# xmed-lab/GL-Fusion

Hardware: AMD Instinct MI355X
Metric: clips/sec fwd+bwd (B=4, 3 views x16x112x112) per GPU, weak scaling (higher is better)
Workload: dtype f32 (amax-scaled split-fp16 x3 MFMA, fp32 accumulate: fp32-equivalent); 1 GPU; C2: (B,V,T,H,W)=(4,3,16,112,112) per GPU, views 1/3/4, fp32 train() fwd + sum-BCE + bwd; global_batch_clips=4, frames_per_view_per_gpu=64, precision=f16x3, parallelism=single GPU, ranks_in_collective=1

## Files before the change

### gl-fusion_amd/csrc/gemm_common.h

```cpp
#pragma once
#include "glf_common.h"

namespace glf {
struct Geo { int n_img, hs, ws, hd, wd, kh, kw, stride, pad, dil; };

struct GemmArgs {
    const float* A; const float* B; const float* bias; float* C;
    int M, N, K, lda, ldb, ldc, taps;
    unsigned tap_mask;
    long long tap_stride_b;
    int gather;
    Geo g;
    long long bsa, bsb, bsc;
    float alpha;
    int accumulate, split;
    int tiles_m, tiles_n;
    int vec_a, vec_b;
    int rect;
    const float* amax_a; const float* amax_b;
    const float* zeros;
    float* amax_c;
    double* colstats;
    float* colmax;
    float* partial;
    unsigned long long* stamps;
    int a_presplit, b_presplit;
    int flags;
    int epi;
    const float* res; long long ld_res;
    int relu;
    const int* seg_tab;
    int seg_kx;
};

constexpr int SEG_MAX = 28, SEG_MAX_BANDS = 7, SEG_MAX_REGIONS = SEG_MAX_BANDS * SEG_MAX_BANDS;
constexpr int SEG_REGION_INTS = 8;
constexpr int SEG_TAB_REGIONS = 64, SEG_TAB_OFFS = SEG_TAB_REGIONS + SEG_REGION_INTS * SEG_MAX_REGIONS;
constexpr int SEG_TAB_INTS = SEG_TAB_OFFS + 2 * SEG_MAX;
static_assert(SEG_TAB_OFFS % 2 == 0, "segment offsets are 8-byte aligned");
constexpr int ZERO_PAGE_FLOATS = 1 << 18;


int precision();
int init_gemm_bf16s_attrs();
bool bf16s_rows_ok(const GemmArgs& a);
bool bf16s_tn_ok(const GemmArgs& a);
int launch_rows_bf16s(const GemmArgs& a, dim3 grid, bool gather, hipStream_t s);
int launch_tn_bf16s(const GemmArgs& a, dim3 grid, bool gather, hipStream_t s);
int init_gemm_f16s_attrs();
int launch_rows_f16s(const GemmArgs& a, dim3 grid, bool gather, int nprod, hipStream_t s);
int launch_tn_f16s(const GemmArgs& a, dim3 grid, bool gather, int nprod, hipStream_t s);
int init_gemm_f16s4_attrs();
bool use_f16s4(const GemmArgs& a);
int launch_rows_f16s4(const GemmArgs& a, dim3 grid, bool gather, int nprod, hipStream_t s);
int launch_amax(const float* x, long long rows, int cols, long long ld, int vec, float* out, hipStream_t s);
int launch_split_packed(const float* x, long long rows, int cols, long long ld, const float* amax, float* out, long long ldo, hipStream_t s);
float* amax_scratch(int n, hipStream_t s);
const float* zero_page();
bool f16s_rows_ok(const GemmArgs& a);
bool f16s_tn_ok(const GemmArgs& a);
int launch_rows_f16s_seg(const GemmArgs& a, const glf_gemm_params* p, int nprod, hipStream_t s);
}

namespace {
using glf::Geo;
using glf::GemmArgs;

typedef float f32x16 __attribute__((ext_vector_type(16)));

constexpr int BM = 128, BN = 128, BK = 32;
constexpr int LD_T = 129;
constexpr int LD_V = 132;
constexpr int NTHREADS = 256;

struct GeoS { int hs, ws, hd, wd, kw, stride, pad, dil; };

__device__ __forceinline__ int map_src(const int hs, const int ws, const int kw, const int stride, const int pad,
                                       const int dil, const int gather, int n, int y, int x, int tap) {
    const int ky = tap / kw, kx = tap - ky * kw;
    int sy, sx;
    if (gather == 1) {
        sy = y * stride - pad + ky * dil;
        sx = x * stride - pad + kx * dil;
        if ((unsigned)sy >= (unsigned)hs || (unsigned)sx >= (unsigned)ws) return -1;
    } else {
        sy = y + pad - ky * dil;
        sx = x + pad - kx * dil;
        if (sy < 0 || sx < 0) return -1;
        if (stride > 1) {
            if ((sy % stride) != 0 || (sx % stride) != 0) return -1;
            sy /= stride; sx /= stride;
        }
        if (sy >= hs || sx >= ws) return -1;
    }
    return (n * hs + sy) * ws + sx;
}

__device__ __forceinline__ float4 ld4(const float* p, int nvalid, bool vec) {
    if (nvalid >= 4 && vec) return *reinterpret_cast<const float4*>(p);
    float4 v = make_float4(0.f, 0.f, 0.f, 0.f);
    if (nvalid > 0) v.x = p[0];
    if (nvalid > 1) v.y = p[1];
    if (nvalid > 2) v.z = p[2];
    if (nvalid > 3) v.w = p[3];
    return v;
}

__host__ __device__ inline void tap_rect(int gather, int tap, int kw, int pad, int dil, int hs, int ws, int hd, int wd,
                                         int& y0, int& y1, int& x0, int& x1) {
    const int ky = tap / kw, kx = tap - ky * kw;
    const int oy = (gather == 1) ? pad - ky * dil : ky * dil - pad;
    const int ox = (gather == 1) ? pad - kx * dil : kx * dil - pad;
    y0 = oy > 0 ? oy : 0;           y1 = hs + oy < hd ? hs + oy : hd;
    x0 = ox > 0 ? ox : 0;           x1 = ws + ox < wd ? ws + ox : wd;
    if (y1 < y0) y1 = y0;
    if (x1 < x0) x1 = x0;
}

__host__ __device__ inline void axis_band(int gather, int b, int d, int h, int& lo, int& hi, unsigned& taps) {
    int e1 = d < h - d ? d : h - d, e2 = d < h - d ? h - d : d;
    e1 = e1 < 0 ? 0 : (e1 > h ? h : e1);
    e2 = e2 < 0 ? 0 : (e2 > h ? h : e2);
    lo = b == 0 ? 0 : (b == 1 ? e1 : e2);
    hi = b == 0 ? e1 : (b == 1 ? e2 : h);
    const unsigned first = gather == 1 ? 0b110u : 0b011u, last = gather == 1 ? 0b011u : 0b110u;
    taps = b == 0 ? first : (b == 2 ? last : (d <= h - d ? 0b111u : 0b010u));
}
__host__ __device__ inline void region_of(int gather, int r, int d, int hd, int wd, int& y0, int& y1, int& x0, int& x1, unsigned& mask) {
    const int cell = (int)((0x8620'7531'4ull >> (4 * r)) & 0xf);
    unsigned ty, tx;
    axis_band(gather, cell / 3, d, hd, y0, y1, ty);
    axis_band(gather, cell % 3, d, wd, x0, x1, tx);
    mask = 0;
    for (int ky = 0; ky < 3; ++ky)
        for (int kx = 0; kx < 3; ++kx)
            if (((ty >> ky) & 1u) && ((tx >> kx) & 1u)) mask |= 1u << (ky * 3 + kx);
}

__device__ __forceinline__ float4 keep_if(bool c, const float4 v) {
// ... 71 lines not shown
```

### gl-fusion_amd/csrc/gemm_f16s.hip

```cpp
#include "gemm_common.h"
#include "split_f16.h"
#include <cstdlib>
#include <cstring>
#include <mutex>
#include <vector>

namespace {
using glf::SEG_TAB_REGIONS; using glf::SEG_REGION_INTS; using glf::SEG_TAB_OFFS;

#define GLF_MFMA_F16(a, b, c) __builtin_amdgcn_mfma_f32_32x32x16_f16(a, b, c, 0, 0, 0)
#define GLF_ROW3(c0, c1, m0, m1, ah, al, b0h, b0l, b1h, b1l)  \
    c0 = GLF_MFMA_F16(ah, b0h, c0);                         \
    c1 = GLF_MFMA_F16(ah, b1h, c1);                         \
    if (NP == 3) {                                          \
        m0 = GLF_MFMA_F16(al, b0h, m0);                     \
        m1 = GLF_MFMA_F16(al, b1h, m1);                     \
        m0 = GLF_MFMA_F16(ah, b0l, m0);                     \
        m1 = GLF_MFMA_F16(ah, b1l, m1);                     \
    }

constexpr int BM8 = 256;
constexpr int NT8 = 512;
constexpr int WAVE_ROWS = 4;
#ifndef GLF_IL_ALL
// ... 1179 lines not shown
#if defined(GLF_STAMPS) && GLF_STAMPS == 2
    wg_t2 = __builtin_amdgcn_s_memtime();
#endif

    const bool atomic = !args.partial && ((p_split > 1) || p_accumulate);
    const int col_l = lane & 31, row_l = 4 * (lane >> 5);
    float cmax = 0.f;
    auto emit = [&](const f32x16& acc, int ti, int tj) {
        const int col = tn * BN + wn + 32 * tj + col_l;
        if (col >= pN) return;
#pragma unroll
        for (int r = 0; r < 16; ++r) {
            const int row = tm * TM8 + wm + 32 * ti + (r & 3) + 8 * (r >> 2) + row_l;
            if (row < pM) {
                float* dst = C + (long long)row * ldc_e + col;
                const float v = p_alpha * acc[r];
                if (atomic) atomicAdd(dst, v); else { *dst = v; cmax = fmaxf(cmax, fabsf(v)); }
            }
        }
    };
    emit(c00 + m00 * 0x1p-11f, 0, 0); emit(c01 + m01 * 0x1p-11f, 0, 1);
    emit(c10 + m10 * 0x1p-11f, 1, 0); emit(c11 + m11 * 0x1p-11f, 1, 1);
    if (args.amax_c && !atomic && !args.partial) {
#pragma unroll
        for (int o = 32; o > 0; o >>= 1) cmax = fmaxf(cmax, __shfl_xor(cmax, o, 64));
        if (lane == 0 && cmax > *reinterpret_cast<volatile float*>(args.amax_c))
            atomicMax(reinterpret_cast<unsigned*>(args.amax_c), __float_as_uint(cmax));
    }
#if defined(GLF_STAMPS) && GLF_STAMPS == 2
    if (args.stamps != nullptr && blockIdx.x == gridDim.x / 2 && blockIdx.z == 0 && blockIdx.y == 0) {
        __builtin_amdgcn_s_waitcnt(0);
        const unsigned long long wg_t3 = __builtin_amdgcn_s_memtime();
        if (lane == 0) {
            unsigned long long* d_ = args.stamps + 64 + wave * 4;
            d_[0] = wg_t0; d_[1] = wg_t1; d_[2] = wg_t2; d_[3] = wg_t3; if (wave == 0) args.stamps[63] = (unsigned long long)ntiles;
        }
    }
#endif
}

__global__ __launch_bounds__(256) void amax_kernel(const float* __restrict__ x, long long rows, int cols, long long ld,
                                                   int vec, unsigned* __restrict__ out) {
    const int c4n = vec ? cols >> 2 : 0;
    const long long total4 = rows * c4n;
    float m = 0.f;
    for (long long i = (long long)blockIdx.x * blockDim.x + threadIdx.x; i < total4; i += (long long)gridDim.x * blockDim.x) {
        const long long r = i / c4n;
        const int c = (int)(i - r * c4n) * 4;
        const float4 v = *reinterpret_cast<const float4*>(x + r * ld + c);
        m = fmaxf(fmaxf(m, fmaxf(fabsf(v.x), fabsf(v.y))), fmaxf(fabsf(v.z), fabsf(v.w)));
    }
    const int tail = cols - 4 * c4n;
    if (tail) {
        for (long long i = (long long)blockIdx.x * blockDim.x + threadIdx.x; i < rows * tail; i += (long long)gridDim.x * blockDim.x) {
            const long long r = i / tail;
            m = fmaxf(m, fabsf(x[r * ld + (cols - tail) + (int)(i - r * tail)]));
        }
    }
#pragma unroll
    for (int o = 32; o > 0; o >>= 1) m = fmaxf(m, __shfl_xor(m, o));
    __shared__ float sm[4];
    if ((threadIdx.x & 63) == 0) sm[threadIdx.x >> 6] = m;
    __syncthreads();
    if (threadIdx.x == 0) {
        m = fmaxf(fmaxf(sm[0], sm[1]), fmaxf(sm[2], sm[3]));
        if (m > 0.f) atomicMax(out, __float_as_uint(m));
    }
}

__global__ __launch_bounds__(256) void split_packed_kernel(const float* __restrict__ x, long long rows, int cols4, long long ld,
                                                           const float* __restrict__ amax, float* __restrict__ out, long long ldo) {
    float sc, inv;
    pow2_scale(amax, sc, inv);
    const long long total = rows * cols4;
    for (long long i = (long long)blockIdx.x * blockDim.x + threadIdx.x; i < total; i += (long long)gridDim.x * blockDim.x) {
        const long long r = i / cols4;
        const int c = (int)(i - r * cols4) * 4;
        const SplitH s = split4h(*reinterpret_cast<const float4*>(x + r * ld + c), sc);
        const float2 h = __builtin_bit_cast(float2, s.h), l = __builtin_bit_cast(float2, s.l);
        *reinterpret_cast<float4*>(out + r * ldo + c) = make_float4(h.x, h.y, l.x, l.y);
    }
}

}

namespace glf {

int launch_split_packed(const float* x, long long rows, int cols, long long ld, const float* amax, float* out, long long ldo, hipStream_t s) {
    const long long total = rows * (cols / 4);
    long long blocks = (total + 255) / 256;
    if (blocks > 8192) blocks = 8192;
    hipLaunchKernelGGL(split_packed_kernel, dim3((unsigned)blocks), dim3(256), 0, s, x, rows, cols / 4, ld, amax, out, ldo);
    return check_launch("split_f16_packed");
}

int init_gemm_f16s_attrs() {
    hipError_t e;
#define SET_ATTR(fn, bytes)                                                                              \
    e = hipFuncSetAttribute(reinterpret_cast<const void*>(fn), hipFuncAttributeMaxDynamicSharedMemorySize, (int)(bytes)); \
    if (e != hipSuccess) return fail(GLF_ERR_LAUNCH, "hipFuncSetAttribute(" #fn "): %s", hipGetErrorString(e));
#define SET_ROWS(G, NP_, PA_, PB_) SET_ATTR((gemm_rows_f16s8_kernel<G, NP_, PB_, PA_>), SMEM_ROWS_H8) SET_ATTR((gemm_rows_f16s8_kernel<G, NP_, PB_, PA_, true>), SMEM_ROWS_H8)
#define SET_TN(G, NP_, PA_, PB_) SET_ATTR((gemm_tn_f16s_kernel<G, NP_, PA_, PB_>), SMEM_TN_H) SET_ATTR((gemm_tn_f16s_kernel<G, NP_, PA_, PB_, true>), SMEM_TN_H) \
                                 SET_ATTR((gemm_tn_f16s8_kernel<G, NP_, PA_, PB_>), SMEM_TN_H8)
#define SET_ALL(G, NP_) SET_ROWS(G, NP_, false, false) SET_ROWS(G, NP_, true, false) SET_ROWS(G, NP_, false, true) SET_ROWS(G, NP_, true, true) \
                        SET_TN(G, NP_, false, false) SET_TN(G, NP_, true, false) SET_TN(G, NP_, false, true) SET_TN(G, NP_, true, true)
    SET_ALL(false, 3) SET_ALL(true, 3) SET_ALL(false, 1) SET_ALL(true, 1)
    SET_ATTR((gemm_rows_f16s8_kernel<false, 3, true, true, false, true>), SMEM_ROWS_H8)
    SET_ATTR((gemm_rows_f16s8_kernel<false, 1, true, true, false, true>), SMEM_ROWS_H8)
#undef SET_ALL
#undef SET_TN
#undef SET_ROWS
#undef SET_ATTR
    return init_gemm_f16s4_attrs();
}

bool f16s_rows_ok(const GemmArgs& a) {
    return a.vec_a && a.vec_b && (a.K % BK) == 0 && a.K >= BK && a.K <= ZERO_PAGE_FLOATS && zero_page() != nullptr;
}
bool f16s_tn_ok(const GemmArgs& a) {
    return a.vec_a && a.vec_b && (a.M % 4) == 0 && (a.N % 4) == 0 && a.M >= 4 && a.N >= 4 &&
           a.M <= ZERO_PAGE_FLOATS && a.N <= ZERO_PAGE_FLOATS && zero_page() != nullptr;
}

#ifdef GLF_STAMPS
static void* stamps_buffer() {
    static void* p = [] { void* q = nullptr; (void)hipMalloc(&q, 8192); (void)hipMemset(q, 0, 8192); return q; }();
    return p;
}
extern "C" int glf_debug_stamps(void* host_out) {
    (void)hipDeviceSynchronize();
    return (int)hipMemcpy(host_out, stamps_buffer(), 8192, hipMemcpyDeviceToHost);
}
#endif

int launch_rows_f16s(const GemmArgs& a0, dim3 grid, bool gather, int nprod, hipStream_t s) {
    if (use_f16s4(a0)) return launch_rows_f16s4(a0, grid, gather, nprod, s);
    GemmArgs a = a0;
    a.zeros = zero_page();
    long long tiles_m = (a.M + BM8 - 1) / BM8;
    if (a.rect == 2) {
        tiles_m = 0;
        for (int r = 0; r < 9; ++r) {
            int y0, y1, x0, x1;
            unsigned rm;
            region_of(a.gather, r, a.g.dil, a.g.hd, a.g.wd, y0, y1, x0, x1, rm);
            if (rm & a.tap_mask) tiles_m += ((long long)a.g.n_img * (y1 - y0) * (x1 - x0) + BM8 - 1) / BM8;
        }
        if (tiles_m == 0) return GLF_OK;
    } else if (a.rect) {
        tiles_m = 0;
        for (unsigned mm = a.tap_mask; mm; mm &= mm - 1) {
            const int t = __builtin_ctz(mm);
            int y0, y1, x0, x1;
            tap_rect(a.gather, t, a.g.kw, a.g.pad, a.g.dil, a.g.hs, a.g.ws, a.g.hd, a.g.wd, y0, y1, x0, x1);
            tiles_m += ((long long)a.g.n_img * (y1 - y0) * (x1 - x0) + BM8 - 1) / BM8;
        }
    }
    a.tiles_m = (int)tiles_m;
    dim3 g2((unsigned)(tiles_m * a.tiles_n), 1, grid.z);
    const int group_m = (a.rect == 0 && a.tiles_n >= 8) ? 4 : 0;
    a.flags = (group_m & 0xff) << 8;
    const bool pa = a.a_presplit != 0, pb = a.b_presplit != 0;
#ifdef GLF_STAMPS
    a.partial = reinterpret_cast<float*>(stamps_buffer());
#endif
#define GLF_LAUNCH_ROWS(G, NP_, PA_, PB_)                                                                                  \
    { if (a.epi) hipLaunchKernelGGL((gemm_rows_f16s8_kernel<G, NP_, PB_, PA_, true>), g2, dim3(NT8), SMEM_ROWS_H8, s, a); \
      else hipLaunchKernelGGL((gemm_rows_f16s8_kernel<G, NP_, PB_, PA_>), g2, dim3(NT8), SMEM_ROWS_H8, s, a); }
#define GLF_ROWS_P(G, NP_)                                                                     \
    { if (pa && pb) GLF_LAUNCH_ROWS(G, NP_, true, true) else if (pa) GLF_LAUNCH_ROWS(G, NP_, true, false) \
      else if (pb) GLF_LAUNCH_ROWS(G, NP_, false, true) else GLF_LAUNCH_ROWS(G, NP_, false, false) }
    if (nprod == 3) { if (gather) GLF_ROWS_P(true, 3) else GLF_ROWS_P(false, 3) }
    else { if (gather) GLF_ROWS_P(true, 1) else GLF_ROWS_P(false, 1) }
#undef GLF_ROWS_P
#undef GLF_LAUNCH_ROWS
    return check_launch("gemm_nt(f16x3, 256x128)");
// ... 182 lines not shown
```

### gl-fusion_amd/csrc/gemm_f32.hip

```cpp
#include "gemm_common.h"

namespace {

#define GLF_LD(x) (x)
#define GLF_MMA_KTILE(LDA_, LDB_, a_s, b_s, MID)                                                              \
    {                                                                                                         \
        constexpr int NS_ = BK / 2, HEAD_ = NS_ - 4;                                                          \
        f32x16 t00 = {0}, t01 = {0}, t10 = {0}, t11 = {0};                                                    \
        float a0_[2], a1_[2], b0_[2], b1_[2];                                                                 \
        float ta0_[4], ta1_[4], tb0_[4], tb1_[4];                                                             \
        a0_[0] = GLF_LD((a_s)[0]); a1_[0] = GLF_LD((a_s)[32]); b0_[0] = GLF_LD((b_s)[0]); b1_[0] = GLF_LD((b_s)[32]); \
        _Pragma("unroll") for (int st = 0; st < HEAD_; ++st) {                                                \
            const int cur = st & 1, nxt = cur ^ 1;                                                            \
            if (st + 1 < HEAD_) {                                                                             \
                a0_[nxt] = GLF_LD((a_s)[(2 * st + 2) * LDA_]); a1_[nxt] = GLF_LD((a_s)[(2 * st + 2) * LDA_ + 32]); \
                b0_[nxt] = GLF_LD((b_s)[(2 * st + 2) * LDB_]); b1_[nxt] = GLF_LD((b_s)[(2 * st + 2) * LDB_ + 32]); \
            } else {                                                                                          \
                _Pragma("unroll") for (int q = 0; q < 4; ++q) {                                               \
                    ta0_[q] = GLF_LD((a_s)[(2 * (HEAD_ + q)) * LDA_]); ta1_[q] = GLF_LD((a_s)[(2 * (HEAD_ + q)) * LDA_ + 32]); \
                    tb0_[q] = GLF_LD((b_s)[(2 * (HEAD_ + q)) * LDB_]); tb1_[q] = GLF_LD((b_s)[(2 * (HEAD_ + q)) * LDB_ + 32]); \
                }                                                                                             \
            }                                                                                                 \
            __builtin_amdgcn_sched_barrier(0);              \
            t00 = __builtin_amdgcn_mfma_f32_32x32x2f32(a0_[cur], b0_[cur], t00, 0, 0, 0);                     \
// ... 716 lines not shown
    }
    if (amax_c) {
#pragma unroll
        for (int o = 32; o > 0; o >>= 1) cmax = fmaxf(cmax, __shfl_xor(cmax, o, 64));
        if ((threadIdx.x & 63) == 0 && cmax > 0.f) atomicMax(reinterpret_cast<unsigned*>(amax_c), __float_as_uint(cmax));
    }
}

constexpr size_t SMEM_ROWS_NT = (2 * BK * LD_T + 2 * BK * LD_T) * sizeof(float) + 16;
constexpr size_t SMEM_ROWS_NN = (2 * BK * LD_T + 2 * BK * LD_V) * sizeof(float) + 16;
constexpr size_t SMEM_TN = (4 * BK * LD_V) * sizeof(float) + 2 * 32 * sizeof(int);

}

namespace glf {
int init_gemm_attrs() {
    hipError_t e;
#define SET_ATTR(fn, bytes)                                                                              \
    e = hipFuncSetAttribute(reinterpret_cast<const void*>(fn), hipFuncAttributeMaxDynamicSharedMemorySize, (int)(bytes)); \
    if (e != hipSuccess) return fail(GLF_ERR_LAUNCH, "hipFuncSetAttribute(" #fn "): %s", hipGetErrorString(e));
    SET_ATTR((gemm_rows_kernel<0, false>), SMEM_ROWS_NT)
    SET_ATTR((gemm_rows_kernel<0, true>), SMEM_ROWS_NT)
    SET_ATTR((gemm_rows_kernel<1, false>), SMEM_ROWS_NN)
    SET_ATTR((gemm_rows_kernel<1, true>), SMEM_ROWS_NN)
    SET_ATTR((gemm_tn_kernel<false>), SMEM_TN)
    SET_ATTR((gemm_tn_kernel<true>), SMEM_TN)
#undef SET_ATTR
    if (int rc = init_gemm_bf16s_attrs()) return rc;
    return init_gemm_f16s_attrs();
}
}

namespace {
int self_amax(GemmArgs& a, const glf_gemm_params* p, bool tn, hipStream_t s) {
    if (a.amax_a && a.amax_b) return GLF_OK;
    float* slots = glf::amax_scratch(2, s);
    GLF_REQUIRE(slots != nullptr, GLF_ERR_WORKSPACE, "gemm(f16x3): no amax scratch");
    hipError_t e = hipMemsetAsync(slots, 0, 2 * sizeof(float), s);
    if (e != hipSuccess) return glf::fail(GLF_ERR_LAUNCH, "hipMemsetAsync(amax): %s", hipGetErrorString(e));
    const long long src_rows = p->gather ? (long long)p->n_img * p->hs * p->ws : 0;
    for (int b = 0; b < p->batch; ++b) {
        if (!a.amax_a) {
            const long long rows = tn ? p->K : (p->gather ? src_rows : p->M);
            const int cols = tn ? p->M : p->K;
            if (int rc = glf::launch_amax(a.A + b * a.bsa, rows, cols, p->lda, a.vec_a, slots, s)) return rc;
        }
        if (!a.amax_b) {
            if (tn) {
                const long long rows = p->gather ? src_rows : p->K;
                if (int rc = glf::launch_amax(a.B + b * a.bsb, rows, p->N, p->ldb, a.vec_b, slots + 1, s)) return rc;
            } else {
                for (unsigned mm = p->tap_mask; mm; mm &= mm - 1) {
                    const int t = __builtin_ctz(mm);
                    if (int rc = glf::launch_amax(a.B + b * a.bsb + t * a.tap_stride_b, p->N, p->K, p->ldb, a.vec_b, slots + 1, s)) return rc;
                }
            }
        }
    }
    if (!a.amax_a) a.amax_a = slots;
    if (!a.amax_b) a.amax_b = slots + 1;
    return GLF_OK;
}
}

extern "C" int glf_amax(const float* x, int64_t rows, int cols, int64_t ld, float* out, glf_stream_t stream) {
    if (int rc = glf::ensure_init()) return rc;
    GLF_REQUIRE(x && out, GLF_ERR_NULL, "amax: null argument");
    GLF_REQUIRE(rows > 0 && cols > 0 && ld >= cols, GLF_ERR_BAD_SHAPE, "amax: bad extents");
    hipError_t e = hipMemsetAsync(out, 0, sizeof(float), glf::S(stream));
    if (e != hipSuccess) return glf::fail(GLF_ERR_LAUNCH, "hipMemsetAsync(amax): %s", hipGetErrorString(e));
    return glf::launch_amax(x, rows, cols, ld, aligned16(x) && (ld % 4 == 0), out, glf::S(stream));
}

extern "C" int glf_split_f16_packed(const float* x, int64_t rows, int cols, int64_t ld, const float* amax, float* out, int64_t ldo,
                                    glf_stream_t stream) {
    if (int rc = glf::ensure_init()) return rc;
    GLF_REQUIRE(x && amax && out, GLF_ERR_NULL, "split_f16_packed: null argument");
    GLF_REQUIRE(rows > 0 && cols > 0 && cols % 4 == 0 && ld % 4 == 0 && ldo % 4 == 0 && ld >= cols && ldo >= cols, GLF_ERR_BAD_SHAPE,
                "split_f16_packed: cols and the row strides must be multiples of 4");
    GLF_REQUIRE(aligned16(x) && aligned16(out), GLF_ERR_BAD_SHAPE, "split_f16_packed: x and out must be 16-byte aligned");
    return glf::launch_split_packed(x, rows, cols, ld, amax, out, ldo, glf::S(stream));
}

constexpr int SK_COLS = 2;
__global__ __launch_bounds__(256) void gemm_skinny_nt_kernel(const float* __restrict__ A, const float* __restrict__ B, const float* __restrict__ bias,
                                                            float* __restrict__ C, int M, int N, int K, int lda, int ldb, int ldc, float alpha,
                                                            int accumulate, float* __restrict__ amax_c) {
    const int tid = threadIdx.x, kl = tid & 3, m = tid >> 2;
    const int n0 = blockIdx.x * SK_COLS;
    const float* a = A + (long long)min(m, M - 1) * lda + 4 * kl;
    const float* b[SK_COLS];
#pragma unroll
    for (int j = 0; j < SK_COLS; ++j) b[j] = B + (long long)min(n0 + j, N - 1) * ldb + 4 * kl;
    float acc[SK_COLS] = {};
    int k = 0;
    for (; k + 64 <= K; k += 64) {
        float4 av[4], bv[SK_COLS][4];
#pragma unroll
        for (int u = 0; u < 4; ++u) av[u] = *reinterpret_cast<const float4*>(a + k + 16 * u);
#pragma unroll
        for (int j = 0; j < SK_COLS; ++j)
#pragma unroll
            for (int u = 0; u < 4; ++u) bv[j][u] = *reinterpret_cast<const float4*>(b[j] + k + 16 * u);
#pragma unroll
        for (int j = 0; j < SK_COLS; ++j)
#pragma unroll
            for (int u = 0; u < 4; ++u)
                acc[j] += av[u].x * bv[j][u].x + av[u].y * bv[j][u].y + av[u].z * bv[j][u].z + av[u].w * bv[j][u].w;
    }
    for (; k < K; k += 16) {
        const float4 av = *reinterpret_cast<const float4*>(a + k);
#pragma unroll
        for (int j = 0; j < SK_COLS; ++j) {
            const float4 bv = *reinterpret_cast<const float4*>(b[j] + k);
            acc[j] += av.x * bv.x + av.y * bv.y + av.z * bv.z + av.w * bv.w;
        }
    }
    float cmax = 0.f;
#pragma unroll
    for (int j = 0; j < SK_COLS; ++j) {
        float v = acc[j];
        v += __shfl_xor(v, 1);
        v += __shfl_xor(v, 2);
        if (kl == 0 && m < M && n0 + j < N) {
            v = v * alpha + (bias ? bias[n0 + j] : 0.f);
            float* c = C + (long long)m * ldc + n0 + j;
            if (accumulate) v += *c;
            *c = v;
            cmax = fmaxf(cmax, fabsf(v));
        }
    }
    if (amax_c) {
#pragma unroll
        for (int o = 32; o > 0; o >>= 1) cmax = fmaxf(cmax, __shfl_xor(cmax, o));
        if ((tid & 63) == 0 && cmax > 0.f) atomicMax(reinterpret_cast<unsigned*>(amax_c), __float_as_uint(cmax));
    }
}

extern "C" int glf_gemm_nt(const float* A, const float* B, const float* bias, float* C,
                           const glf_gemm_params* p, glf_stream_t stream) {
    if (int rc = glf::ensure_init()) return rc;
    if (int rc = validate(p, A, B, C)) return rc;
    if (p->gather) GLF_REQUIRE((long long)p->n_img * p->hd * p->wd == p->M, GLF_ERR_BAD_SHAPE,
                               "gemm_nt: M (%d) != n_img*hd*wd", p->M);
    if (p->tap_mask == 0) return glf::fail(GLF_ERR_BAD_SHAPE, "gemm_nt: empty tap_mask");
    GemmArgs a = make_args(A, B, bias, C, p);
    const int prec = call_precision(p);
    a.vec_a = aligned16(A) && (p->lda % 4 == 0) && (p->batch_stride_a % 4 == 0);
    a.vec_b = aligned16(B) && (p->ldb % 4 == 0) && (p->batch_stride_b % 4 == 0) && (p->tap_stride_b % 4 == 0);
    dim3 grid(a.tiles_m * a.tiles_n, 1, p->batch);
    if (p->nseg != 0) {
        GLF_REQUIRE(p->nseg >= 1 && p->nseg <= GLF_SEG_MAX && p->seg != nullptr, GLF_ERR_UNSUPPORTED, "glf_gemm_nt: nseg must be in [1, %d] with a segment list", GLF_SEG_MAX);
        GLF_REQUIRE(prec >= 2 && glf::f16s_rows_ok(a) && p->a_presplit && p->b_presplit && p->amax_a && p->amax_b, GLF_ERR_UNSUPPORTED,
                    "glf_gemm_nt: segments need precision 3 / 4, the aligned fast path and both operands pre-split with their amax");
        GLF_REQUIRE(!p->gather && p->taps == 1 && !p->rect && !p->accumulate && !p->colstats && !p->colmax && p->batch == 1, GLF_ERR_UNSUPPORTED,
                    "glf_gemm_nt: segments extend a plain NT launch (no gather, rect, accumulate, colstats or batch)");
        GLF_REQUIRE(p->n_img > 0 && p->hd > 0 && p->wd > 0 && (long long)p->n_img * p->hd * p->wd == p->M && p->K <= p->lda && p->N <= p->ldc,
                    GLF_ERR_BAD_SHAPE, "glf_gemm_nt: segments need M (%d) == n_img*hd*wd, K <= lda and N <= ldc", p->M);
        GLF_REQUIRE(p->seg_kx >= BK && p->seg_kx % BK == 0 && (long long)p->K + (long long)p->nseg * p->seg_kx <= p->ldb &&
                    (long long)p->K + (long long)p->nseg * p->seg_kx + BK <= glf::ZERO_PAGE_FLOATS, GLF_ERR_UNSUPPORTED,
                    "glf_gemm_nt: segments need seg_kx %% 32 == 0 and K + nseg * seg_kx <= ldb, < 2^18");
        for (int i = 0; i < p->nseg; ++i)
            GLF_REQUIRE(p->seg[3 * i + 2] >= 0 && p->seg[3 * i + 2] % 4 == 0 && p->seg[3 * i + 2] + p->seg_kx <= p->lda, GLF_ERR_UNSUPPORTED,
                        "glf_gemm_nt: segment %d: acol must be a multiple of 4 with acol + seg_kx <= lda", i);
        return glf::launch_rows_f16s_seg(a, p, prec == 2 ? 3 : 1, glf::S(stream));
    }
// ... 194 lines not shown
```

### gl-fusion_amd/csrc/norm.hip

```cpp
#include "stream_common.h"
#include "split_f16.h"

using namespace glf;

namespace {

constexpr int RT = 256;
constexpr int MAX_SLICES = 1024;

__host__ __device__ inline int n_slices_c(int rows, int c) {
    int s = (rows + 31) / 32;
    int cap = 524288 / (c > 0 ? c : 1);
    if (cap < 128) cap = 128;
    if (cap > MAX_SLICES) cap = MAX_SLICES;
    return s < 1 ? 1 : (s > cap ? cap : s);
}

struct Coef { const float* mean; const float* invstd; const float* gamma; const float* beta; };

struct OpStats {
    const float* x; int ldx;
    __device__ void operator()(int r, int c, float4& a, float4& b) const {
        a = *reinterpret_cast<const float4*>(x + (long long)r * ldx + c);
        b = make_float4(a.x * a.x, a.y * a.y, a.z * a.z, a.w * a.w);
// ... 234 lines not shown
                const unsigned m = RM == 1 ? op.mask[row * op.c4 + cc] : 15u;
                fold(row, qa, qa2, qx, qy, m);
            }
        }
        const int ncol = tpr * 4;
        for (int pass = 0; pass < (cmax ? 2 : 1); ++pass) {
            if (rl < rpp) {
                const float4 u = pass == 0 ? sa : mg, v = pass == 0 ? sb : mx;
                float* d0 = sh + (0 * rpp + rl) * ncol + ct * 4;
                float* d1 = sh + (1 * rpp + rl) * ncol + ct * 4;
                d0[0] = u.x; d0[1] = u.y; d0[2] = u.z; d0[3] = u.w;
                d1[0] = v.x; d1[1] = v.y; d1[2] = v.z; d1[3] = v.w;
            }
            __syncthreads();
            for (int idx = tid; idx < 2 * ncol; idx += RT) {
                const int st = idx / ncol, col = idx - st * ncol;
                const int gc = cb * 4 + col;
                if (gc < c) {
                    if (pass == 0) {
                        double d = 0;
                        for (int q = 0; q < rpp; ++q) d += sh[(st * rpp + q) * ncol + col];
                        atomicAdd(sums + st * c + gc, d);
                    } else {
                        float m = 0.f;
                        for (int q = 0; q < rpp; ++q) m = fmaxf(m, sh[(st * rpp + q) * ncol + col]);
                        if (m > 0.f) atomicMax(reinterpret_cast<unsigned*>(cmax + st * c + gc), __float_as_uint(m));
                    }
                }
            }
            __syncthreads();
        }
    }
}

constexpr int FIN_CH = 16, FIN_LANES = 16;

__device__ __forceinline__ void fold_partials(const double* __restrict__ partial, int slices, int c, int ch, int lane,
                                              double& s, double& q, double* sh) {
    s = 0; q = 0;
    if (ch < c) {
        double s1 = 0, q1 = 0, s2 = 0, q2 = 0, s3 = 0, q3 = 0;
        int i = lane;
        for (; i + 3 * FIN_LANES < slices; i += 4 * FIN_LANES) {
            s += partial[(long long)i * c + ch];                     q += partial[(long long)(slices + i) * c + ch];
            s1 += partial[(long long)(i + FIN_LANES) * c + ch];      q1 += partial[(long long)(slices + i + FIN_LANES) * c + ch];
            s2 += partial[(long long)(i + 2 * FIN_LANES) * c + ch];  q2 += partial[(long long)(slices + i + 2 * FIN_LANES) * c + ch];
            s3 += partial[(long long)(i + 3 * FIN_LANES) * c + ch];  q3 += partial[(long long)(slices + i + 3 * FIN_LANES) * c + ch];
        }
        for (; i < slices; i += FIN_LANES) {
            s += partial[(long long)i * c + ch];
            q += partial[(long long)(slices + i) * c + ch];
        }
        s += (s1 + s2) + s3; q += (q1 + q2) + q3;
    }
    const int t = threadIdx.x;
    sh[t] = s; sh[256 + t] = q;
    __syncthreads();
    if (lane == 0) {
        for (int l = 1; l < FIN_LANES; ++l) { s += sh[t + l * FIN_CH]; q += sh[256 + t + l * FIN_CH]; }
    }
}

__global__ __launch_bounds__(256) void bn_stats_finalize(const double* __restrict__ partial, int slices, int c, int rows, float eps,
                                                         float momentum, float* mean, float* invstd, float* rmean, float* rvar, long long* nbt) {
    __shared__ double sh[512];
    const int cx = threadIdx.x % FIN_CH, lane = threadIdx.x / FIN_CH;
    const int ch = blockIdx.x * FIN_CH + cx;
    double s, q;
    fold_partials(partial, slices, c, ch, lane, s, q, sh);
    if (lane != 0 || ch >= c) return;
    if (ch == 0 && nbt) *nbt += 1;
    const double m = s / rows;
    double var = q / rows - m * m;
    if (var < 0) var = 0;
    mean[ch] = (float)m;
    invstd[ch] = (float)(1.0 / sqrt(var + (double)eps));
    if (rmean) {
        const double unb = rows > 1 ? var * rows / (rows - 1) : var;
        rmean[ch] = (1.f - momentum) * rmean[ch] + momentum * (float)m;
        rvar[ch] = (1.f - momentum) * rvar[ch] + momentum * (float)unb;
    }
}

__global__ __launch_bounds__(256) void sum_finalize(const double* __restrict__ partial, int slices, int c, float* out_a, float* out_b) {
    __shared__ double sh[512];
    const int cx = threadIdx.x % FIN_CH, lane = threadIdx.x / FIN_CH;
    const int ch = blockIdx.x * FIN_CH + cx;
    double s, q;
    fold_partials(partial, slices, c, ch, lane, s, q, sh);
    if (lane != 0 || ch >= c) return;
    if (out_a) out_a[ch] = (float)s;
    if (out_b) out_b[ch] = (float)q;
}

__global__ __launch_bounds__(256) void bnbwd_finalize(const double* __restrict__ partial, const float* __restrict__ pmax, int slices, int c,
                                                      const float* __restrict__ gamma, const float* __restrict__ invstd, float inv_n,
                                                      int training, float* out_a, float* out_b, float* __restrict__ bound,
                                                      float* __restrict__ keep) {
    __shared__ double sh[512];
    __shared__ float shm[512];
    const int cx = threadIdx.x % FIN_CH, lane = threadIdx.x / FIN_CH;
    const int ch = blockIdx.x * FIN_CH + cx;
    double s, q;
    fold_partials(partial, slices, c, ch, lane, s, q, sh);
    float mg = 0.f, mx = 0.f;
    if (ch < c) {
        float g1 = 0.f, x1 = 0.f, g2 = 0.f, x2 = 0.f, g3 = 0.f, x3 = 0.f;
        int i = lane;
        for (; i + 3 * FIN_LANES < slices; i += 4 * FIN_LANES) {
            mg = fmaxf(mg, pmax[(long long)i * c + ch]);                      mx = fmaxf(mx, pmax[(long long)(slices + i) * c + ch]);
            g1 = fmaxf(g1, pmax[(long long)(i + FIN_LANES) * c + ch]);        x1 = fmaxf(x1, pmax[(long long)(slices + i + FIN_LANES) * c + ch]);
            g2 = fmaxf(g2, pmax[(long long)(i + 2 * FIN_LANES) * c + ch]);    x2 = fmaxf(x2, pmax[(long long)(slices + i + 2 * FIN_LANES) * c + ch]);
            g3 = fmaxf(g3, pmax[(long long)(i + 3 * FIN_LANES) * c + ch]);    x3 = fmaxf(x3, pmax[(long long)(slices + i + 3 * FIN_LANES) * c + ch]);
        }
        for (; i < slices; i += FIN_LANES) {
            mg = fmaxf(mg, pmax[(long long)i * c + ch]);
            mx = fmaxf(mx, pmax[(long long)(slices + i) * c + ch]);
        }
        mg = fmaxf(fmaxf(mg, g1), fmaxf(g2, g3)); mx = fmaxf(fmaxf(mx, x1), fmaxf(x2, x3));
    }
    shm[threadIdx.x] = mg; shm[256 + threadIdx.x] = mx;
    __syncthreads();
    if (lane != 0 || ch >= c) return;
    for (int l = 1; l < FIN_LANES; ++l) { mg = fmaxf(mg, shm[threadIdx.x + l * FIN_CH]); mx = fmaxf(mx, shm[256 + threadIdx.x + l * FIN_CH]); }
    if (out_a) out_a[ch] = (float)s;
    if (out_b) out_b[ch] = (float)q;
    if (keep) { keep[ch] = (float)s; keep[c + ch] = (float)q; }
    const float k = fabsf(gamma[ch] * invstd[ch]);
    const float b = 1.0001f * k * (training ? mg + inv_n * (fabsf((float)s) + mx * fabsf((float)q)) : mg);
    if (b > 0.f && b < 3.0e38f) atomicMax(reinterpret_cast<unsigned*>(bound), __float_as_uint(b));
}

__global__ void bn_replay_kernel(const float* __restrict__ mean, const float* __restrict__ invstd, int rows, float eps, float momentum,
                                 float* rmean, float* rvar, long long* nbt, int c) {
    const int ch = blockIdx.x * blockDim.x + threadIdx.x;
    if (ch == 0 && nbt) *nbt += 1;
    if (ch >= c) return;
    const double is = (double)invstd[ch];
    double var = 1.0 / (is * is) - (double)eps;
    if (var < 0) var = 0;
    const double unb = rows > 1 ? var * rows / (rows - 1) : var;
    rmean[ch] = (1.f - momentum) * rmean[ch] + momentum * mean[ch];
    rvar[ch] = (1.f - momentum) * rvar[ch] + momentum * (float)unb;
}

__global__ void bn_eval_coeffs_kernel(const float* rm, const float* rv, float eps, float* mean, float* invstd, int c) {
    const int ch = blockIdx.x * blockDim.x + threadIdx.x;
    if (ch >= c) return;
    mean[ch] = rm[ch];
    invstd[ch] = 1.0f / sqrtf(rv[ch] + eps);
}

constexpr int APPLY_TPR = 16, APPLY_TPR_WIDE = 64;
constexpr int APPLY_MAXCOL = APPLY_TPR_WIDE * 4;

struct ColGrid { int tpr, cblocks, slices; };
inline ColGrid col_grid(int rows, int c) {
    const int c4 = c / 4;
    const int tpr = c4 >= APPLY_TPR_WIDE ? APPLY_TPR_WIDE : (c4 < APPLY_TPR ? c4 : APPLY_TPR);
    const int rpp = 256 / tpr;
    const int cblocks = (c4 + tpr - 1) / tpr;
    long long s = stream_grid((long long)rows * c4, 256) / cblocks;
    const int smax = (rows + rpp - 1) / rpp;
    if (s > smax) s = smax;
    if (s < 1) s = 1;
    return {tpr, cblocks, (int)s};
}
inline dim3 col_dim(const ColGrid& g) { return dim3((unsigned)g.slices * (unsigned)g.cblocks); }

struct ColLane { int cb, slice, cc, c0, r, r1, rpp; bool live; };
__device__ __forceinline__ ColLane col_lane(int rows, int c4, int tpr, int cblocks, int slices) {
    ColLane L;
    L.rpp = 256 / tpr;
    const int ct = threadIdx.x % tpr, rl = threadIdx.x / tpr;
    L.cb = blockIdx.x % cblocks; L.slice = blockIdx.x / cblocks;
    const int per = (rows + slices - 1) / slices;
    const int r0 = L.slice * per;
    L.r1 = min(rows, r0 + per);
    L.r = r0 + rl;
    L.cc = L.cb * tpr + ct; L.c0 = L.cc * 4;
    L.live = L.cc < c4 && rl < L.rpp;
    return L;
}

template <bool RES>
__device__ __forceinline__ float bn_apply_rows(const ColLane& L, const float* __restrict__ x, int ldx, const float* __restrict__ res, int ldr,
                                               float* __restrict__ y, int ldy, const float4 mu, const float4 is, const float4 ga, const float4 be,
                                               int c4, int relu, unsigned char* __restrict__ mask, bool packed, float sc) {
    float am = 0.f;
    const int c0 = L.c0, cc = L.cc, rpp = L.rpp;
    auto emit = [&](long long row, const float4 xx, const float4 rr) __attribute__((always_inline)) {
        float4 o = make_float4(bn_val(xx.x, mu.x, is.x, ga.x, be.x), bn_val(xx.y, mu.y, is.y, ga.y, be.y),
                               bn_val(xx.z, mu.z, is.z, ga.z, be.z), bn_val(xx.w, mu.w, is.w, ga.w, be.w));
        if (RES) { o.x += rr.x; o.y += rr.y; o.z += rr.z; o.w += rr.w; }
        if (mask) mask[row * c4 + cc] = (unsigned char)((o.x > 0.f) | ((o.y > 0.f) << 1) | ((o.z > 0.f) << 2) | ((o.w > 0.f) << 3));
        if (relu) { o.x = fmaxf(o.x, 0.f); o.y = fmaxf(o.y, 0.f); o.z = fmaxf(o.z, 0.f); o.w = fmaxf(o.w, 0.f); }
        if (packed) {
            const SplitH sp = split4h(o, sc);
            const float2 h = __builtin_bit_cast(float2, sp.h), l = __builtin_bit_cast(float2, sp.l);
            o = make_float4(h.x, h.y, l.x, l.y);
        } else {
            am = fmaxf(fmaxf(am, fmaxf(fabsf(o.x), fabsf(o.y))), fmaxf(fabsf(o.z), fabsf(o.w)));
        }
        *reinterpret_cast<float4*>(y + row * ldy + c0) = o;
    };
    int r = L.r;
    for (; r + 3 * rpp < L.r1; r += 4 * rpp) {
        float4 qx[4], qr[4];
#pragma unroll
        for (int u = 0; u < 4; ++u) {
            const long long row = r + u * rpp;
            qx[u] = *reinterpret_cast<const float4*>(x + row * ldx + c0);
            if (RES) qr[u] = *reinterpret_cast<const float4*>(res + row * ldr + c0);
// ... 226 lines not shown
    const long long base = (long long)row * c;
    float4 u[LN_NV];
    float s = 0.f;
#pragma unroll
    for (int v = 0; v < LN_NV; ++v) {
        const int cc = lane + 64 * v;
        if (cc < c4) {
            const int ch = cc * 4;
            const float4 ww = *reinterpret_cast<const float4*>(w + base + ch);
            const float4 xx = *reinterpret_cast<const float4*>(x + base + ch);
            const float4 mu = *reinterpret_cast<const float4*>(bn.mean + ch);
            const float4 is = *reinterpret_cast<const float4*>(bn.invstd + ch);
            const float4 ga = *reinterpret_cast<const float4*>(bn.gamma + ch);
            const float4 be = *reinterpret_cast<const float4*>(bn.beta + ch);
            u[v] = make_float4((ww.x - mu.x) * is.x * ga.x + be.x + xx.x, (ww.y - mu.y) * is.y * ga.y + be.y + xx.y,
                               (ww.z - mu.z) * is.z * ga.z + be.z + xx.z, (ww.w - mu.w) * is.w * ga.w + be.w + xx.w);
            s += (u[v].x + u[v].y) + (u[v].z + u[v].w);
        } else {
            u[v] = make_float4(0.f, 0.f, 0.f, 0.f);
        }
    }
    float mean, rstd;
    if (!BWD) {
        mean = wave_sum(s) / c;
        float q = 0.f;
#pragma unroll
        for (int v = 0; v < LN_NV; ++v)
            if (lane + 64 * v < c4) {
                const float a = u[v].x - mean, b = u[v].y - mean, cc2 = u[v].z - mean, d = u[v].w - mean;
                q += (a * a + b * b) + (cc2 * cc2 + d * d);
            }
        rstd = 1.0f / sqrtf(wave_sum(q) / c + eps);
        if (lane == 0) { row_mean[row] = mean; row_rstd[row] = rstd; }
        float am = 0.f;
#pragma unroll
        for (int v = 0; v < LN_NV; ++v) {
            const int cc = lane + 64 * v;
            if (cc < c4) {
                const int ch = cc * 4;
                const float4 g = *reinterpret_cast<const float4*>(ln_g + ch);
                const float4 b = *reinterpret_cast<const float4*>(ln_b + ch);
                const float4 o = make_float4((u[v].x - mean) * rstd * g.x + b.x, (u[v].y - mean) * rstd * g.y + b.y,
                                             (u[v].z - mean) * rstd * g.z + b.z, (u[v].w - mean) * rstd * g.w + b.w);
                *reinterpret_cast<float4*>(z + base + ch) = o;
                am = fmaxf(fmaxf(am, fmaxf(fabsf(o.x), fabsf(o.y))), fmaxf(fabsf(o.z), fabsf(o.w)));
            }
        }
        if (amax_out) {
#pragma unroll
            for (int o = 32; o > 0; o >>= 1) am = fmaxf(am, __shfl_xor(am, o, 64));
            if (lane == 0 && am > *reinterpret_cast<volatile float*>(amax_out)) atomicMax(reinterpret_cast<unsigned*>(amax_out), __float_as_uint(am));
        }
    } else {
        mean = row_mean[row]; rstd = row_rstd[row];
        float4 gz[LN_NV];
        float s1 = 0.f, s2 = 0.f;
#pragma unroll
        for (int v = 0; v < LN_NV; ++v) {
            const int cc = lane + 64 * v;
            if (cc < c4) {
                const int ch = cc * 4;
                const float4 d = *reinterpret_cast<const float4*>(dz + base + ch);
                const float4 g = *reinterpret_cast<const float4*>(ln_g + ch);
                gz[v] = make_float4(d.x * g.x, d.y * g.y, d.z * g.z, d.w * g.w);
                u[v] = make_float4((u[v].x - mean) * rstd, (u[v].y - mean) * rstd, (u[v].z - mean) * rstd, (u[v].w - mean) * rstd);
                s1 += (gz[v].x + gz[v].y) + (gz[v].z + gz[v].w);
                s2 += (gz[v].x * u[v].x + gz[v].y * u[v].y) + (gz[v].z * u[v].z + gz[v].w * u[v].w);
            } else {
                gz[v] = make_float4(0.f, 0.f, 0.f, 0.f);
            }
        }
        const float m1 = wave_sum(s1) / c, m2 = wave_sum(s2) / c;
#pragma unroll
        for (int v = 0; v < LN_NV; ++v) {
            const int cc = lane + 64 * v;
            if (cc < c4)
                *reinterpret_cast<float4*>(du + base + cc * 4) =
                    make_float4(rstd * (gz[v].x - m1 - u[v].x * m2), rstd * (gz[v].y - m1 - u[v].y * m2),
                                rstd * (gz[v].z - m1 - u[v].z * m2), rstd * (gz[v].w - m1 - u[v].w * m2));
        }
    }
}

template <class Op>
int launch_colreduce(Op op, int rows, int c, double* ws, hipStream_t s) {
    const int slices = n_slices_c(rows, c);
    const int c4 = c / 4, tpr = c4 < RT ? c4 : RT;
    hipLaunchKernelGGL((colreduce_kernel<Op>), dim3(slices, (c4 + tpr - 1) / tpr), dim3(RT), 0, s, op, rows, c, slices, ws);
    return glf::check_launch("colreduce");
}

}

extern "C" size_t glf_bn_workspace(int rows, int c) {
    return (size_t)3 * MAX_SLICES * (size_t)(c > 0 ? c : 0) + (size_t)2 * (c > 0 ? c : 0);
}

#define REQ_C4(c) GLF_REQUIRE((c) > 0 && ((c) % 4) == 0, GLF_ERR_BAD_SHAPE, "channel count must be a positive multiple of 4 (got %d)", (c))
#define REQ_LD(ld, name) GLF_REQUIRE(((ld) % 4) == 0, GLF_ERR_BAD_SHAPE, name " must be a multiple of 4")

extern "C" int glf_bn_stats(const float* x, int ldx, int rows, int c, float eps, float momentum,
                            float* mean, float* invstd, float* running_mean, float* running_var,
                            int64_t* num_batches_tracked, double* workspace, glf_stream_t s) {
    if (int rc = glf::ensure_init()) return rc;
    GLF_REQUIRE(x && mean && invstd && workspace, GLF_ERR_NULL, "bn_stats: null argument");
    GLF_REQUIRE(rows > 0, GLF_ERR_BAD_SHAPE, "bn_stats: rows must be > 0");
    REQ_C4(c); REQ_AL(x, "x"); REQ_LD(ldx, "ldx");
    GLF_REQUIRE((running_mean == nullptr) == (running_var == nullptr), GLF_ERR_NULL, "bn_stats: running_mean/var must both be set or both NULL");
    if (int rc = launch_colreduce(OpStats{x, ldx}, rows, c, workspace, glf::S(s))) return rc;
    hipLaunchKernelGGL(bn_stats_finalize, dim3((c + FIN_CH - 1) / FIN_CH), dim3(256), 0, glf::S(s), workspace, n_slices_c(rows, c), c, rows,
                       eps, momentum, mean, invstd, running_mean, running_var, reinterpret_cast<long long*>(num_batches_tracked));
    return glf::check_launch("bn_stats_finalize");
}

extern "C" int glf_bn_stats_from_sums(const double* sums, int rows, int c, float eps, float momentum, float* mean, float* invstd,
                                      float* running_mean, float* running_var, int64_t* num_batches_tracked, glf_stream_t s) {
    if (int rc = glf::ensure_init()) return rc;
    GLF_REQUIRE(sums && mean && invstd, GLF_ERR_NULL, "bn_stats_from_sums: null argument");
    GLF_REQUIRE(rows > 0 && c > 0, GLF_ERR_BAD_SHAPE, "bn_stats_from_sums: rows and c must be > 0");
    GLF_REQUIRE((running_mean == nullptr) == (running_var == nullptr), GLF_ERR_NULL, "bn_stats_from_sums: running_mean/var must both be set or both NULL");
    hipLaunchKernelGGL(bn_stats_finalize, dim3((c + FIN_CH - 1) / FIN_CH), dim3(256), 0, glf::S(s), sums, 1, c, rows,
                       eps, momentum, mean, invstd, running_mean, running_var, reinterpret_cast<long long*>(num_batches_tracked));
    return glf::check_launch("bn_stats_from_sums");
}

extern "C" int glf_bn_replay_running(const float* mean, const float* invstd, int rows, int c, float eps, float momentum,
                                     float* running_mean, float* running_var, int64_t* num_batches_tracked, glf_stream_t s) {
    if (int rc = glf::ensure_init()) return rc;
    GLF_REQUIRE(mean && invstd && running_mean && running_var, GLF_ERR_NULL, "bn_replay_running: null argument");
    GLF_REQUIRE(rows > 0 && c > 0, GLF_ERR_BAD_SHAPE, "bn_replay_running: rows and c must be > 0");
    hipLaunchKernelGGL(bn_replay_kernel, dim3((c + 255) / 256), dim3(256), 0, glf::S(s), mean, invstd, rows, eps, momentum,
                       running_mean, running_var, reinterpret_cast<long long*>(num_batches_tracked), c);
    return glf::check_launch("bn_replay_running");
}

extern "C" int glf_bn_eval_coeffs(const float* rm, const float* rv, float eps, float* mean, float* invstd, int c, glf_stream_t s) {
    GLF_REQUIRE(rm && rv && mean && invstd, GLF_ERR_NULL, "bn_eval_coeffs: null argument");
    GLF_REQUIRE(c > 0, GLF_ERR_BAD_SHAPE, "bn_eval_coeffs: c must be > 0");
    hipLaunchKernelGGL(bn_eval_coeffs_kernel, dim3((c + 255) / 256), dim3(256), 0, glf::S(s), rm, rv, eps, mean, invstd, c);
    return glf::check_launch("bn_eval_coeffs");
}

extern "C" int glf_bn_apply(const float* x, int ldx, const float* residual, int ldr, float* y, int ldy,
                            const float* mean, const float* invstd, const float* gamma, const float* beta,
                            int rows, int c, int relu, float* amax_out, uint8_t* relu_mask, glf_stream_t s) {
    if (int rc = glf::ensure_init()) return rc;
    GLF_REQUIRE(x && y && mean && invstd && gamma && beta, GLF_ERR_NULL, "bn_apply: null argument");
    GLF_REQUIRE(rows > 0, GLF_ERR_BAD_SHAPE, "bn_apply: rows must be > 0");
    REQ_C4(c); REQ_AL(x, "x"); REQ_AL(y, "y"); REQ_LD(ldx, "ldx"); REQ_LD(ldy, "ldy");
    if (residual) { REQ_AL(residual, "residual"); REQ_LD(ldr, "ldr"); }
    const ColGrid g = col_grid(rows, c);
#define GLF_BNF(RES_) hipLaunchKernelGGL((bn_apply_kernel<RES_>), col_dim(g), dim3(256), 0, glf::S(s), x, ldx, residual, ldr, y, ldy, \
                                         Coef{mean, invstd, gamma, beta}, rows, c / 4, g.tpr, g.cblocks, g.slices, relu, amax_out, relu_mask)
    if (residual) GLF_BNF(true); else GLF_BNF(false);
#undef GLF_BNF
    return glf::check_launch("bn_apply");
}

extern "C" int glf_bn_apply_from_sums(const float* x, int ldx, const float* residual, int ldr, float* y, int ldy, const double* sums,
                                      int rows, int c, float eps, float momentum, const float* gamma, const float* beta,
                                      float* mean, float* invstd, float* running_mean, float* running_var, int64_t* num_batches_tracked,
                                      int relu, float* amax_out, uint8_t* relu_mask, const float* colmax, glf_stream_t s) {
    if (int rc = glf::ensure_init()) return rc;
    GLF_REQUIRE(x && y && sums && mean && invstd && gamma && beta, GLF_ERR_NULL, "bn_apply_from_sums: null argument");
    GLF_REQUIRE(!colmax || (amax_out && !residual && y != x), GLF_ERR_BAD_SHAPE, "bn_apply_from_sums: the packed output (colmax) needs amax_out, no residual and y != x");
    GLF_REQUIRE(rows > 0, GLF_ERR_BAD_SHAPE, "bn_apply_from_sums: rows must be > 0");
    REQ_C4(c); REQ_AL(x, "x"); REQ_AL(y, "y"); REQ_LD(ldx, "ldx"); REQ_LD(ldy, "ldy");
    GLF_REQUIRE(c <= APPLY_MAX_C, GLF_ERR_UNSUPPORTED, "bn_apply_from_sums: C must be <= %d (use glf_bn_stats_from_sums + glf_bn_apply)", APPLY_MAX_C);
    GLF_REQUIRE((running_mean == nullptr) == (running_var == nullptr), GLF_ERR_NULL, "bn_apply_from_sums: running_mean/var must both be set or both NULL");
    if (residual) { REQ_AL(residual, "residual"); REQ_LD(ldr, "ldr"); }
    const ColGrid g = col_grid(rows, c);
#define GLF_BNF(RES_) hipLaunchKernelGGL((bn_apply_sums_kernel<RES_>), col_dim(g), dim3(256), 0, glf::S(s), x, ldx, residual, ldr, y, ldy, sums, rows, c, \
                                         eps, momentum, gamma, beta, mean, invstd, running_mean, running_var,                                      \
                                         reinterpret_cast<long long*>(num_batches_tracked), g.tpr, g.cblocks, g.slices, relu, amax_out, relu_mask, colmax)
    if (residual) GLF_BNF(true); else GLF_BNF(false);
#undef GLF_BNF
    return glf::check_launch("bn_apply_from_sums");
}

extern "C" int glf_bn_bwd(const float* dy, int lddy, const float* x, int ldx, const float* y, int ldy,
                          const float* mean, const float* invstd, const float* gamma, const float* beta,
                          float* dx, int lddx, float* dres, int lddres, float* dgamma, float* dbeta,
                          int rows, int c, int relu, int training, double* workspace, float* amax_out, int packed_dx,
                          const uint8_t* relu_mask, const float* dy2, int lddy2, double* fused_sums, glf_stream_t s) {
    if (int rc = glf::ensure_init()) return rc;
    GLF_REQUIRE(dy && x && mean && invstd && gamma && dx && (workspace || fused_sums), GLF_ERR_NULL, "bn_bwd: null argument");
    if (relu_mask) y = nullptr;
    GLF_REQUIRE(!packed_dx || amax_out, GLF_ERR_NULL, "bn_bwd: packed_dx needs amax_out (a zeroed device float that receives the bound the image is scaled with)");
    GLF_REQUIRE(!relu || y || beta || relu_mask, GLF_ERR_NULL, "bn_bwd: relu != 0 needs relu_mask, y (the forward output) or beta (to recompute its sign from x)");
    GLF_REQUIRE(rows > 0, GLF_ERR_BAD_SHAPE, "bn_bwd: rows must be > 0");
    REQ_C4(c); REQ_AL(dy, "dy"); REQ_AL(x, "x"); REQ_AL(dx, "dx"); REQ_LD(lddy, "lddy"); REQ_LD(ldx, "ldx"); REQ_LD(lddx, "lddx");
    if (relu && y) { REQ_AL(y, "y"); REQ_LD(ldy, "ldy"); }
    if (dres) { REQ_AL(dres, "dres"); REQ_LD(lddres, "lddres"); }
    if (dy2) { REQ_AL(dy2, "dy2"); REQ_LD(lddy2, "lddy2"); }
    const OpBnBwd op{dy, lddy, x, ldx, y, ldy, mean, invstd, gamma, beta, relu, relu_mask, c / 4, dy2, lddy2};
    const ColGrid ag = col_grid(rows, c);
    BwdApply ap{dy, lddy, x, ldx, y, ldy, Coef{mean, invstd, gamma, beta}, nullptr, nullptr, dx, lddx, dres, lddres,
                rows, c, ag.tpr, ag.cblocks, ag.slices, training, 1.0f / (float)rows,
                amax_out, packed_dx, relu_mask, dy2, lddy2, nullptr, nullptr, nullptr, nullptr};
    const int phase = packed_dx >= 2 ? packed_dx : 0;
    GLF_REQUIRE(packed_dx >= 0 && packed_dx <= 3, GLF_ERR_BAD_SHAPE, "bn_bwd: packed_dx must be 0 .. 3");
    GLF_REQUIRE(!phase || (workspace && fused_sums), GLF_ERR_NULL, "bn_bwd: packed_dx = 2 / 3 needs the workspace and fused_sums (2 c floats kept from half 2 to half 3)");
    GLF_REQUIRE(phase != 2 || (dgamma && dbeta), GLF_ERR_NULL, "bn_bwd: packed_dx = 2 needs dgamma and dbeta");
    float* keep = phase ? reinterpret_cast<float*>(fused_sums) : (float*)nullptr;
    if (!phase && fused_sums && c <= APPLY_MAX_C) {
        float* fmax = reinterpret_cast<float*>(fused_sums + (size_t)2 * c);
        const int fs = fused_slices(rows, c);
        const int c4 = c / 4, tpr = c4 < FUSED_TPR ? c4 : FUSED_TPR;
        const dim3 rgrid(fs, (c4 + tpr - 1) / tpr);
        float* rmax = packed_dx ? fmax : (float*)nullptr;
        const int rm = !op.relu ? 0 : (op.mask ? 1 : (op.y ? 3 : 2));
        const bool wres = dy2 && dres;
        GLF_REQUIRE(!wres || (dres != dy && dres != dy2 && dres != x), GLF_ERR_BAD_SHAPE, "bn_bwd: dres must not alias dy, dy2 or x");
#define GLF_BNR(H2, RM_, WR) hipLaunchKernelGGL((bnbwd_reduce_atomic_kernel<H2, RM_, WR>), rgrid, dim3(RT), 0, glf::S(s), op, rows, c, fs, fused_sums, rmax, \
                                                (WR) ? dres : (float*)nullptr, lddres)
        if (wres) { if (rm == 0) GLF_BNR(true, 0, true); else if (rm == 1) GLF_BNR(true, 1, true); else if (rm == 2) GLF_BNR(true, 2, true); else GLF_BNR(true, 3, true); }
        else if (op.dy2) { if (rm == 0) GLF_BNR(true, 0, false); else if (rm == 1) GLF_BNR(true, 1, false); else if (rm == 2) GLF_BNR(true, 2, false); else GLF_BNR(true, 3, false); }
        else { if (rm == 0) GLF_BNR(false, 0, false); else if (rm == 1) GLF_BNR(false, 1, false); else if (rm == 2) GLF_BNR(false, 2, false); else GLF_BNR(false, 3, false); }
#undef GLF_BNR
        if (int rc = glf::check_launch("bn_bwd_reduce(fused)")) return rc;
        ap.fsums = fused_sums; ap.fmax = fmax; ap.out_dbeta = dbeta; ap.out_dgamma = dgamma;
        if (wres) {
            ap.dy = dres; ap.lddy = lddres; ap.dy2 = nullptr; ap.mask = nullptr; ap.y = nullptr; ap.dres = nullptr;
            return launch_bwd_apply(ap, 0, glf::S(s));
        }
        return launch_bwd_apply(ap, relu, glf::S(s));
    }
    GLF_REQUIRE(workspace, GLF_ERR_NULL, "bn_bwd: the three-launch form needs the workspace");
    const int slices = n_slices_c(rows, c);
    float* sums = reinterpret_cast<float*>(workspace + (size_t)2 * slices * c);
    float* s_dy = dbeta ? dbeta : sums;
    float* s_dyx = dgamma ? dgamma : sums + c;
    if (phase == 3) {
        s_dy = keep; s_dyx = keep + c;
    } else if (packed_dx) {
        float* pmax = reinterpret_cast<float*>(workspace + (size_t)2 * slices * c + (size_t)2 * c);
        const int c4 = c / 4, tpr = c4 < RT ? c4 : RT;
        hipLaunchKernelGGL(bnbwd_reduce_kernel, dim3(slices, (c4 + tpr - 1) / tpr), dim3(RT), 0, glf::S(s), op, rows, c, slices, workspace, pmax);
        if (int rc = glf::check_launch("bn_bwd_reduce")) return rc;
        hipLaunchKernelGGL(bnbwd_finalize, dim3((c + FIN_CH - 1) / FIN_CH), dim3(256), 0, glf::S(s), workspace, pmax, slices, c, gamma, invstd,
                           1.0f / (float)rows, training, s_dy, s_dyx, amax_out, keep);
    } else {
        if (int rc = launch_colreduce(op, rows, c, workspace, glf::S(s))) return rc;
        hipLaunchKernelGGL(sum_finalize, dim3((c + FIN_CH - 1) / FIN_CH), dim3(256), 0, glf::S(s), workspace, slices, c, s_dy, s_dyx);
    }
    if (int rc = glf::check_launch("bn_bwd_finalize")) return rc;
    if (phase == 2) return GLF_OK;
    ap.sum_dy = s_dy; ap.sum_dyx = s_dyx;
    return launch_bwd_apply(ap, relu, glf::S(s));
}

extern "C" int glf_colsum(const float* dy, int lddy, float* db, int rows, int c, double* workspace, glf_stream_t s) {
    if (int rc = glf::ensure_init()) return rc;
    GLF_REQUIRE(dy && db && workspace, GLF_ERR_NULL, "colsum: null argument");
    GLF_REQUIRE(rows > 0, GLF_ERR_BAD_SHAPE, "colsum: rows must be > 0");
    REQ_C4(c); REQ_AL(dy, "dy"); REQ_LD(lddy, "lddy");
    if (int rc = launch_colreduce(OpColsum{dy, lddy}, rows, c, workspace, glf::S(s))) return rc;
    hipLaunchKernelGGL(sum_finalize, dim3((c + FIN_CH - 1) / FIN_CH), dim3(256), 0, glf::S(s), workspace, n_slices_c(rows, c), c, db, (float*)nullptr);
    return glf::check_launch("colsum_finalize");
}

extern "C" int glf_bn_res_ln_fwd(const float* w, const float* x, const float* bn_mean, const float* bn_invstd,
                                 const float* bn_gamma, const float* bn_beta, const float* ln_gamma,
                                 const float* ln_beta, float ln_eps, float* z, float* row_mean, float* row_rstd,
                                 int rows, int c, float* amax_out, glf_stream_t s) {
    if (int rc = glf::ensure_init()) return rc;
    GLF_REQUIRE(w && x && bn_mean && bn_invstd && bn_gamma && bn_beta && ln_gamma && ln_beta && z && row_mean && row_rstd,
                GLF_ERR_NULL, "bn_res_ln_fwd: null argument");
    GLF_REQUIRE(rows > 0, GLF_ERR_BAD_SHAPE, "bn_res_ln_fwd: rows must be > 0");
    REQ_C4(c); GLF_REQUIRE(c <= 64 * 4 * LN_NV, GLF_ERR_UNSUPPORTED, "bn_res_ln: C must be <= %d", 64 * 4 * LN_NV);
    REQ_AL(w, "w"); REQ_AL(x, "x"); REQ_AL(z, "z");
    hipLaunchKernelGGL((bn_res_ln_kernel<false>), dim3((rows + 3) / 4), dim3(256), 0, glf::S(s), w, x,
                       Coef{bn_mean, bn_invstd, bn_gamma, bn_beta}, ln_gamma, ln_beta, ln_eps, z, row_mean, row_rstd,
                       (const float*)nullptr, (float*)nullptr, rows, c, amax_out);
    return glf::check_launch("bn_res_ln_fwd");
}

extern "C" int glf_bn_res_ln_bwd(const float* dz, const float* w, const float* x, const float* bn_mean,
                                 const float* bn_invstd, const float* bn_gamma, const float* bn_beta,
                                 const float* ln_gamma, const float* row_mean, const float* row_rstd,
                                 float* du, float* dln_gamma, float* dln_beta, int rows, int c,
                                 double* workspace, glf_stream_t s) {
    if (int rc = glf::ensure_init()) return rc;
    GLF_REQUIRE(dz && w && x && bn_mean && bn_invstd && bn_gamma && bn_beta && ln_gamma && row_mean && row_rstd && du &&
                dln_gamma && dln_beta && workspace, GLF_ERR_NULL, "bn_res_ln_bwd: null argument");
    GLF_REQUIRE(rows > 0, GLF_ERR_BAD_SHAPE, "bn_res_ln_bwd: rows must be > 0");
    REQ_C4(c); GLF_REQUIRE(c <= 64 * 4 * LN_NV, GLF_ERR_UNSUPPORTED, "bn_res_ln: C must be <= %d", 64 * 4 * LN_NV);
    REQ_AL(dz, "dz"); REQ_AL(w, "w"); REQ_AL(x, "x"); REQ_AL(du, "du");
    const Coef bn{bn_mean, bn_invstd, bn_gamma, bn_beta};
    hipLaunchKernelGGL((bn_res_ln_kernel<true>), dim3((rows + 3) / 4), dim3(256), 0, glf::S(s), w, x, bn, ln_gamma,
                       (const float*)nullptr, 0.f, (float*)nullptr, const_cast<float*>(row_mean), const_cast<float*>(row_rstd),
                       dz, du, rows, c, (float*)nullptr);
    if (int rc = glf::check_launch("bn_res_ln_bwd")) return rc;
    if (int rc = launch_colreduce(OpLnParam{dz, w, x, bn, row_mean, row_rstd, c}, rows, c, workspace, glf::S(s))) return rc;
    hipLaunchKernelGGL(sum_finalize, dim3((c + FIN_CH - 1) / FIN_CH), dim3(256), 0, glf::S(s), workspace, n_slices_c(rows, c), c, dln_gamma, dln_beta);
    return glf::check_launch("ln_param_finalize");
}
```

### gl-fusion_amd/fusion.py

```python
from __future__ import annotations

import ctypes as C
import os
import weakref
from types import SimpleNamespace

import torch
from torch.autograd import Function
from torch.autograd.function import once_differentiable

from ._lib import AttnPairParams, AttnParams, check, lib
from .ops import (_chk, _contig, _p, _stream, _tn_split, _ws, _wimage, _registry, WJ_COPY, stats_slot, bnbwd_slot, amax_of, amax_slot, colsum, gemm, set_amax, split_mode,
                  transpose2d, weight_T, weight_packed, nt_presplit_ok, tn_presplit_ok, act_packed, packed_hit, pick, zeros, _ones4)


FUSED_SOFTMAX = os.environ.get("GLF_FUSED_SOFTMAX", "1") != "0"
EXACT_KCHUNK = int(os.environ.get("GLF_EXACT_KCHUNK", "256"))
_gemm = gemm


def gemm(mode, A, B, Cm, **kw):
    K = kw["K"]
    if split_mode() or mode == "tn" or EXACT_KCHUNK <= 0 or K <= EXACT_KCHUNK or kw.get("taps", 1) != 1:
        return _gemm(mode, A, B, Cm, **kw)
    first = True
    for k0 in range(0, K, EXACT_KCHUNK):
        kk = dict(kw)
        kk["K"] = min(EXACT_KCHUNK, K - k0)
        if not first:
            kk["bias"] = None
            kk["accumulate"] = True
        _gemm(mode, A[..., k0:], B[..., k0:] if mode == "nt" else B[..., k0:, :], Cm, **kk)
        first = False
CHUNKED_SOFTMAX = os.environ.get("GLF_CHUNKED_SOFTMAX", "1") != "0"
CHUNK_BYTES = int(os.environ.get("GLF_SOFTMAX_CHUNK_BYTES", str(2 << 30)))


def chunked_softmax_ok(ci: int, L: int) -> bool:
    return CHUNKED_SOFTMAX and split_mode() and ci % 32 == 0 and L % 4 == 0


def gaussian_chunked_ok(ci: int) -> bool:
    return ci % 32 == 0


def pair_relu_ok(ci: int) -> bool:
    return ci % 32 == 0 and ci <= 1024


def _frames_per_chunk(n: int, L: int) -> int:
    lp = (L + 31) // 32 * 32
    return max(1, min(n, CHUNK_BYTES // (L * lp * 4)))


def _scores(th, ph, f0, g, L, lp, ci, c3, am_q, S):
    bq = L * c3
    gemm("nt", th[f0 * L:], ph[f0 * L:], S, M=L, N=L, K=ci, lda=c3, ldb=c3, ldc=lp, batch=g, bsa=bq, bsb=bq, bsc=L * lp,
         amax_a=am_q, amax_b=am_q)
    check(lib.glf_softmax_rows_ld(_p(S), g * L, L, lp, _stream()), "softmax_rows_ld")


def _transposed(src, f0, g, L, lp, ci, c3, out):
    check(lib.glf_transpose2d_strided(_p(src[f0 * L:]), c3, L * c3, _p(out), lp, ci * lp, L, ci, lp, g, _stream()), "transpose2d_strided")


def fused_softmax_ok(ci: int) -> bool:
    return FUSED_SOFTMAX and ci % 32 == 0 and ci <= 1024


def _pair_params(n: int, L: int, ci: int, ldg: int, ldy: int, lddy: int, lddg: int) -> AttnPairParams:
    pp = AttnPairParams()
    pp.frames, pp.L, pp.ci = n, L, ci
    pp.ldg, pp.ldy, pp.lddy, pp.lddg = ldg, ldy, lddy, lddg
    return pp


def _attn_params(n: int, L: int, ci: int, ldqkv: int, ldy: int) -> AttnParams:
    ap = AttnParams()
    ap.frames, ap.L, ap.ci = n, L, ci
    ap.ldq = ap.ldk = ap.ldv = ldqkv
    ap.ldy, ap.lddy, ap.ldd = ldy, ldy, ldqkv
    return ap


_qkv_cache = {}


def _qkv_weights(params):
    k = len(params) // 2
    ws_, bs_ = params[:k], params[k:]
    th_w = ws_[0]
    ci, c = th_w.shape[0], th_w.shape[1]
    if ci % 4 != 0:
        Wcat = torch.cat([_contig(t.detach()).view(ci, c) for t in ws_], dim=0)
        bcat = torch.cat([t.detach() for t in bs_], dim=0)
        return Wcat, bcat
    key = id(th_w)
    hit = _qkv_cache.get(key)
    if hit is None or hit[0]() is not th_w or hit[1].device != th_w.device or hit[1].shape != (k * ci, c):
        Wcat = torch.empty(k * ci, c, dtype=torch.float32, device=th_w.device)
# ... 205 lines not shown
        att = _full_softmax_fwd(G, (x2, x2, c, c, am_x), g, y)
    return y, att


def _gaussian_bwd(G, x, qkv, att, y, am_q, dy, am_dy, dqkv, am_dq_slot, du, wf):
    c, g = G.c, _slices(G, qkv)[2]
    x2 = x.view(G.rows, c)
    scores, sink = (x2, x2, c, c, amax_of(x)), (du, du, c, True, None)
    if gaussian_chunked_ok(G.ci):
        _group_softmax_bwd(G, scores, g, am_q, dy, am_dy, dqkv, am_dq_slot, sink)
    else:
        _full_softmax_bwd(G, scores, att, g, am_q, dy, am_dy, dqkv, sink)
    return None, None


def _concatenate_fwd(G, x, qkv, am_x, am_q, wf):
    n, L, ci, c3, rows = G.n, G.L, G.ci, G.c3, G.rows
    th, ph, g = _slices(G, qkv)
    wf_w, wf_b = wf
    if not pair_relu_ok(ci):
        raise RuntimeError(f"TPAVI mode 'concatenate' is built for Ci % 32 == 0, Ci <= 1024 (got {ci})")
    y = torch.empty(rows, ci, **G.f32)
    wrow = _contig(wf_w.detach()).view(2 * ci)
    att = torch.empty(2, rows, **G.f32)
    check(lib.glf_attn_pair_proj_fwd(_p(th), _p(ph), c3, _p(wrow), _p(att[0]), _p(att[1]), rows, ci, _stream()), "attn_pair_proj_fwd")
    pp = _pair_params(n, L, ci, c3, ci, ci, c3)
    check(lib.glf_attn_pair_relu_fwd(_p(att[0]), _p(att[1]), _p(wf_b), _p(g), _p(y), C.byref(pp), _stream()), "attn_pair_relu_fwd")
    return y, att


def _concatenate_bwd(G, x, qkv, att, y, am_q, dy, am_dy, dqkv, am_dq_slot, du, wf):
    n, L, ci, c3, rows = G.n, G.L, G.ci, G.c3, G.rows
    th, ph, g = _slices(G, qkv)
    dth, dph, dg = _slices(G, dqkv)
    wf_w, wf_b = wf
    wrow = _contig(wf_w.detach()).view(2 * ci)
    dab = torch.empty(2, rows, **G.f32)
    dwf_w = torch.empty(2 * ci, **G.f32)
    dwf_b = torch.empty(1, **G.f32)
    pp = _pair_params(n, L, ci, c3, ci, ci, c3)
    nb = int(lib.glf_attn_pair_relu_workspace_bytes(C.byref(pp)))
    ws = torch.empty(nb // 4, **G.f32)
    check(lib.glf_attn_pair_relu_bwd(_p(att[0]), _p(att[1]), _p(wf_b), _p(g), _p(dy), _p(dg), _p(dab[0]), _p(dab[1]), _p(dwf_b),
                                     _p(ws), nb, C.byref(pp), _stream()), "attn_pair_relu_bwd")
    nb = int(lib.glf_attn_pair_proj_workspace_bytes(rows, ci))
    ws = torch.empty(nb // 4, **G.f32)
    check(lib.glf_attn_pair_proj_bwd(_p(th), _p(ph), c3, _p(wrow), _p(dab[0]), _p(dab[1]), _p(dth), _p(dph), c3, _p(dwf_w), _p(ws), nb,
                                     rows, ci, _stream()), "attn_pair_proj_bwd")
    return dwf_w.view(wf_w.shape), dwf_b


_CORES = {"dot": (_dot_fwd, _dot_bwd), "embedded": (_embedded_fwd, _embedded_bwd), "gaussian": (_gaussian_fwd, _gaussian_bwd),
          "concatenate": (_concatenate_fwd, _concatenate_bwd)}


def _split_dgrad(G) -> bool:
    return split_mode() and G.ci % 32 == 0 and G.c % 32 == 0


def _project(G, x, Wcat, bcat):
    rows, c, c3 = G.rows, G.c, G.c3
    qkv = torch.empty(rows, c3, **G.f32)
    am_x = amax_of(x)
    am_q = amax_slot(G.dev)
    am_wc = amax_of(Wcat)
    ok = nt_presplit_ok(c, c, c)
    wb, pb = pick(Wcat, weight_packed(Wcat, Wcat, "w", am_wc) if ok else None, ok)
    xa, pa = pick(x, act_packed(x, am_x) if ok else None, ok)
    gemm("nt", xa, wb, qkv, M=rows, N=c3, K=c, lda=c, ldb=c, ldc=c3, bias=bcat, amax_a=am_x, amax_b=am_wc, amax_c=am_q,
         a_packed=pa, b_packed=pb)
    x_packed = (xa, am_x) if (pa and packed_hit(x, am_x) is not None) else None
    set_amax(qkv, am_q)
    return qkv, am_x, am_q, x_packed


def _project_bwd(G, x, dqkv, Wcat, du, x_packed):
    rows, c, c3 = G.rows, G.c, G.c3
    sp = _tn_split(rows, c3, c, 1)
    if not split_mode():
        sp = max(sp, min((rows + 511) // 512, 65535))
    dWcat = torch.empty(c3, c, **G.f32)
    am_dq = amax_of(dqkv)
    ok = tn_presplit_ok(c3, c, c3, c)
    dq_a, pa = pick(dqkv, act_packed(dqkv, am_dq, True) if ok else None, ok)
    am_x = x_packed[1] if x_packed is not None else amax_of(x)
    xb, pb = pick(x, x_packed[0] if x_packed is not None else None, ok)
    gemm("tn", dq_a, xb, dWcat, M=c3, N=c, K=rows, lda=c3, ldb=c, ldc=c, split=sp, amax_a=am_dq, amax_b=am_x, a_packed=pa, b_packed=pb)
    dbcat = colsum(dqkv, rows, c3)
    if _split_dgrad(G):
        WcatT = weight_T(Wcat, Wcat)
        am_wc = amax_of(Wcat)
        ok = nt_presplit_ok(c3, c3, c3)
        wb, pb = pick(WcatT, weight_packed(WcatT, Wcat, "T2", am_wc), ok)
        da, pa = pick(dqkv, act_packed(dqkv, am_dq, True) if ok else None, ok)
        gemm("nt", da, wb, du, M=rows, N=c, K=c3, lda=c3, ldb=c3, ldc=c, accumulate=True, amax_a=am_dq, amax_b=am_wc,
             a_packed=pa, b_packed=pb)
    else:
        gemm("nn", dqkv, Wcat, du, M=rows, N=c, K=c3, lda=c3, ldb=c, ldc=c, accumulate=True)
    return dWcat, dbcat


def _tail(G, x, y, zW, wz_w, wz_b, bn_g, bn_b, ln_g, ln_b, rmean, rvar, nbt, training, momentum, bn_eps, ln_eps):
    rows, c, ci, dev = G.rows, G.c, G.ci, G.dev
    wz = torch.empty(rows, c, **G.f32)
    am_zw = amax_of(wz_w)
    ok = nt_presplit_ok(ci, ci, ci)
    wb, pb = pick(zW, weight_packed(zW, wz_w, "w", am_zw) if ok else None, ok)
    am_y = amax_of(y)
    ya, pa = pick(y, act_packed(y, am_y) if ok else None, ok)
    fuse_stats = training and split_mode() and nt_presplit_ok(ci, ci, ci) and c % 4 == 0
    sums = stats_slot(c, dev) if fuse_stats else None
    gemm("nt", ya, wb, wz, M=rows, N=c, K=ci, lda=ci, ldb=ci, ldc=c, bias=wz_b, amax_a=am_y, amax_b=am_zw, a_packed=pa, b_packed=pb,
         colstats=sums)
    y_packed = (ya, am_y) if (pa and packed_hit(y, am_y) is not None) else None
    mean = torch.empty(c, **G.f32)
    invstd = torch.empty(c, **G.f32)
    if fuse_stats:
        check(lib.glf_bn_stats_from_sums(_p(sums), rows, c, bn_eps, momentum, _p(mean), _p(invstd), _p(rmean), _p(rvar), _p(nbt),
                                         _stream()), "bn_stats_from_sums")
    elif training:
        check(lib.glf_bn_stats(_p(wz), c, rows, c, bn_eps, momentum, _p(mean), _p(invstd), _p(rmean), _p(rvar), _p(nbt),
                               _p(_ws(rows, c, dev)), _stream()), "bn_stats")
    else:
        check(lib.glf_bn_eval_coeffs(_p(rmean), _p(rvar), bn_eps, _p(mean), _p(invstd), c, _stream()), "bn_eval_coeffs")
    z = torch.empty_like(x)
    rmu = torch.empty(rows, **G.f32)
    rrs = torch.empty(rows, **G.f32)
    am_z = amax_slot(dev)
    check(lib.glf_bn_res_ln_fwd(_p(wz), _p(x), _p(mean), _p(invstd), _p(bn_g), _p(bn_b), _p(ln_g), _p(ln_b), ln_eps,
                                _p(z), _p(rmu), _p(rrs), rows, c, _p(am_z), _stream()), "bn_res_ln_fwd")
    set_amax(z, am_z)
    return z, wz, mean, invstd, rmu, rrs, y_packed


def _tail_bwd(G, dz, x, y, wz, mean, invstd, rmu, rrs, zW, wz_o, bn_g, bn_b, ln_g, training, y_packed):
    rows, c, ci, dev = G.rows, G.c, G.ci, G.dev
    du = torch.empty(rows, c, **G.f32)
    dln_g = torch.empty(c, **G.f32)
    dln_b = torch.empty(c, **G.f32)
    check(lib.glf_bn_res_ln_bwd(_p(dz), _p(wz), _p(x), _p(mean), _p(invstd), _p(bn_g), _p(bn_b), _p(ln_g), _p(rmu), _p(rrs),
                                _p(du), _p(dln_g), _p(dln_b), rows, c, _p(_ws(rows, c, dev)), _stream()), "bn_res_ln_bwd")
    split = _split_dgrad(G)
    dwz = torch.empty(rows, c, **G.f32)
    am_dwz_slot = amax_slot(dev)
    dbn_g = torch.empty(c, **G.f32)
    dbn_b = torch.empty(c, **G.f32)
    dwz_pk = bool(training and split and am_dwz_slot is not None and nt_presplit_ok(c, c, c) and tn_presplit_ok(c, ci, c, ci))
    fused = bnbwd_slot(c, dev) if c <= 4096 else None
    check(lib.glf_bn_bwd(_p(du), c, _p(wz), c, None, c, _p(mean), _p(invstd), _p(bn_g), None, _p(dwz), c, None, c,
                         _p(dbn_g), _p(dbn_b), rows, c, 0, int(training), None if fused is not None else _p(_ws(rows, c, dev)), _p(am_dwz_slot),
                         int(dwz_pk), None, None, 0, _p(fused), _stream()), "bn_bwd")
    set_amax(dwz, am_dwz_slot)
    sp = _tn_split(rows, c, ci, 1)
    if not split_mode():
        sp = max(sp, min((rows + 511) // 512, 65535))
    dzW = torch.empty(c, ci, **G.f32)
    am_dwz = amax_of(dwz)
    ok = tn_presplit_ok(c, ci, c, ci)
    dwz_a, pa = (dwz, True) if dwz_pk else pick(dwz, act_packed(dwz, am_dwz, True) if ok else None, ok)
    am_y = y_packed[1] if y_packed is not None else amax_of(y)
    yb, pb = pick(y, y_packed[0] if y_packed is not None else None, ok)
    gemm("tn", dwz_a, yb, dzW, M=c, N=ci, K=rows, lda=c, ldb=ci, ldc=ci, split=sp, amax_a=am_dwz, amax_b=am_y, a_packed=pa, b_packed=pb)
    dzb = zeros(c, device=dev) if dwz_pk else colsum(dwz, rows, c)
    dy = torch.empty(rows, ci, **G.f32)
    if split:
        am_dy_slot = amax_slot(dev)
        zWT, am_zw = weight_T(zW, wz_o), amax_of(wz_o)
        ok = nt_presplit_ok(c, c, c)
        wb, pb = pick(zWT, weight_packed(zWT, wz_o, "T2", am_zw), ok)
        da, pa = (dwz, True) if dwz_pk else pick(dwz, act_packed(dwz, am_dwz, True) if ok else None, ok)
        gemm("nt", da, wb, dy, M=rows, N=ci, K=c, lda=c, ldb=c, ldc=ci, amax_a=am_dwz, amax_b=am_zw,
             amax_c=am_dy_slot, a_packed=pa, b_packed=pb)
        set_amax(dy, am_dy_slot)
    else:
        gemm("nn", dwz, zW, dy, M=rows, N=ci, K=c, lda=c, ldb=ci, ldc=ci)
    return du, dy, (dzW, dzb, dbn_g, dbn_b, dln_g, dln_b)


class TpaviFn(Function):
    @staticmethod
    def forward(ctx, x, th_w, th_b, ph_w, ph_b, g_w, g_b, wz_w, wz_b, bn_g, bn_b, ln_g, ln_b,
                rmean, rvar, nbt, training: bool, momentum: float, bn_eps: float, ln_eps: float, mode: str, wf_w=None, wf_b=None):
        x, G = _unpack(x, g_w, mode)
        zW = _contig(wz_w.detach()).view(wz_w.shape[0], wz_w.shape[1])
        Wcat, bcat = _qkv_weights((g_w, g_b) if G.npj == 1 else (th_w, ph_w, g_w, th_b, ph_b, g_b))
        qkv, am_x, am_q, ctx.x_packed = _project(G, x, Wcat, bcat)
        ctx.qkv_owner = g_w if G.npj == 1 else th_w
        ctx.wf = (wf_w, wf_b)
        y, att = _CORES[mode][0](G, x, qkv, am_x, am_q, ctx.wf)
        z, wz, mean, invstd, rmu, rrs, ctx.y_packed = _tail(G, x, y, zW, wz_w, wz_b, bn_g, bn_b, ln_g, ln_b, rmean, rvar, nbt,
                                                            training, momentum, bn_eps, ln_eps)
        ctx.save_for_backward(x, qkv, att, y, wz, mean, invstd, rmu, rrs, Wcat, zW, bn_g, bn_b, ln_g)
        ctx.cfg = (G.n, G.L, G.c, G.ci, training, mode, tuple(g_w.shape), tuple(wz_w.shape))
        ctx.owners = (wz_w,)
        return z

    @staticmethod
    @once_differentiable
    def backward(ctx, dz):
        (x, qkv, att, y, wz, mean, invstd, rmu, rrs, Wcat, zW, bn_g, bn_b, ln_g) = ctx.saved_tensors
        n, L, c, ci, training, mode, pshape, zshape = ctx.cfg
        G = _block(n, L, c, ci, mode, dz.device)
        du, dy, (dzW, dzb, dbn_g, dbn_b, dln_g, dln_b) = _tail_bwd(G, _contig(dz), x, y, wz, mean, invstd, rmu, rrs, zW, ctx.owners[0],
                                                                  bn_g, bn_b, ln_g, training, ctx.y_packed)
        dqkv = torch.empty(G.rows, G.c3, **G.f32)
        am_dq_slot = amax_slot(G.dev)
        dwf_w, dwf_b = _CORES[mode][1](G, x, qkv, att, y, amax_of(qkv), dy, amax_of(dy), dqkv, am_dq_slot, du, ctx.wf)
        del dy
        dWcat, dbcat = _project_bwd(G, x, dqkv, Wcat, du, ctx.x_packed)
        return _grads(G, x, du, dWcat, dbcat, pshape, dzW.view(zshape), dzb, dbn_g, dbn_b, dln_g, dln_b, dwf_w, dwf_b)


def tpavi_forward(x5: torch.Tensor, mod) -> torch.Tensor:
    bn = mod.W_z[1]
    training = bn.training
    if training and bn.momentum is None:
        raise RuntimeError("glfusion_amd: cumulative-average BatchNorm (momentum=None) is not built")
    fn = TpaviFn
    if x5.dtype == torch.bfloat16:
        from .fusion16 import Tpavi16Fn
        fn = Tpavi16Fn
    theta, phi = getattr(mod, "theta", None), getattr(mod, "phi", None)
    args = (x5, theta.weight if theta is not None else None, theta.bias if theta is not None else None,
            phi.weight if phi is not None else None, phi.bias if phi is not None else None, mod.g.weight, mod.g.bias,
            mod.W_z[0].weight, mod.W_z[0].bias, bn.weight, bn.bias, mod.norm_layer.weight, mod.norm_layer.bias,
            bn.running_mean, bn.running_var, bn.num_batches_tracked if training else None,
            training, float(bn.momentum or 0.0), float(bn.eps), float(mod.norm_layer.eps), mod.mode)
    wf = mod.W_f[0] if mod.mode == "concatenate" else None
    args += (wf.weight if wf is not None else None, wf.bias if wf is not None else None)
    return fn.apply(*args)
```

### gl-fusion_amd/ops.py

```python
from __future__ import annotations

import ctypes as C
import os
import weakref
from typing import List, Optional, Sequence, Tuple

import torch
from torch.autograd import Function
from torch.autograd.function import once_differentiable

from ._lib import GemmEpilogue, GemmParams, SEG_MAX, TN_OIHW_MAX_TAPS, WeightJob, WJ_AMAX, WJ_COPY, WJ_PACK, WJ_PASSES, WJ_PASS_OF, WJ_TAP_MAJOR, WJ_TAP_MAJOR_T, WJ_TRANSPOSE, WJ_ZERO, check, lib


BF = torch.bfloat16
DT_F32, DT_BF16 = 0, 1


def _is16(t) -> bool:
    return isinstance(t, torch.Tensor) and t.dtype == BF


def _p(t: Optional[torch.Tensor]):
    return None if t is None else C.c_void_p(t.data_ptr())

# ... 568 lines not shown
def weight_packed(layout: torch.Tensor, owner: torch.Tensor, tag: str, amax: Optional[torch.Tensor]) -> Optional[torch.Tensor]:
    if not presplit_ok(layout, amax):
        return None
    im, fresh = _wimage(owner, "pk:" + tag, WJ_PACK, layout, (layout.numel(), 0, 0), lambda: torch.empty_like(layout), amax)
    if fresh:
        cols = layout.shape[-1]
        check(lib.glf_split_f16_packed(_p(layout), layout.numel() // cols, cols, cols, _p(amax), _p(im.dst), cols, _stream()), "split_f16_packed")
    return im.dst


def packed_hit(t: torch.Tensor, amax: Optional[torch.Tensor]) -> Optional[torch.Tensor]:
    hit = getattr(t, "_glf_packed", None)
    if hit is not None and hit[0] == t._version and hit[1] == t.data_ptr() and hit[2] is amax:
        pk, made_on = hit[3], (hit[4] if len(hit) > 4 else None)
        if made_on is not None:
            cur = torch.cuda.current_stream()
            if made_on.cuda_stream != cur.cuda_stream:
                cur.wait_stream(made_on)
                pk.record_stream(cur)
        return pk
    share = getattr(t, "_glf_pack_share", None)
    if share is not None and share[0] is not None and share[0][0] == t.data_ptr() and share[0][1] is amax:
        pk, made_on = share[0][2], share[0][3]
        cur = torch.cuda.current_stream()
        if made_on.cuda_stream != cur.cuda_stream:
            cur.wait_stream(made_on)
            pk.record_stream(cur)
        return pk
    return None


PRESPLIT_KEEP_FRAC = float(os.environ.get("GLF_PRESPLIT_KEEP_FRAC", "0.5"))
PRESPLIT_OFF_FRAC = float(os.environ.get("GLF_PRESPLIT_OFF_FRAC", "0.6"))
_dev_total = {}
_retain_off = {}
_retain_step = {}


def retain_ok(dev) -> bool:
    hit = _retain_step.get(dev)
    if hit is not None:
        return hit
    tot = _dev_total.get(dev)
    if tot is None:
        tot = _dev_total[dev] = torch.cuda.get_device_properties(dev).total_memory
    off = _retain_off.get(dev, 0)
    if off:
        if off == 1 and torch.cuda.memory_allocated(dev) < 0.3 * tot and not torch.cuda.is_current_stream_capturing():
            torch.cuda.empty_cache()
            _retain_off[dev] = 2
        _retain_step[dev] = False
        return False
    r = torch.cuda.memory_reserved(dev)
    if r > PRESPLIT_OFF_FRAC * tot:
        _retain_off[dev] = 1
        _retain_step[dev] = False
        return False
    ok = r < PRESPLIT_KEEP_FRAC * tot
    if ok:
        _retain_step[dev] = True
    return ok


def act_packed(t: torch.Tensor, amax: Optional[torch.Tensor], retain: Optional[bool] = None) -> Optional[torch.Tensor]:
    if not presplit_ok(t, amax):
        return None
    pk = packed_hit(t, amax)
    if pk is not None:
        return pk
    pk = packed_of(t, amax)
    if retain is None:
        retain = retain_ok(t.device)
    if retain:
        try:
            t._glf_packed = (t._version, t.data_ptr(), amax, pk, torch.cuda.current_stream() if STREAMS else None)
        except AttributeError:
            pass
        share = getattr(t, "_glf_pack_share", None)
        if share is not None:
            share[0] = (t.data_ptr(), amax, pk, torch.cuda.current_stream())
    return pk


def nt_presplit_ok(K: int, lda: int, ldb: int) -> bool:
    return _PREC[0] >= 2 and K % 32 == 0 and 32 <= K <= (1 << 18) and lda % 4 == 0 and ldb % 4 == 0


def tn_presplit_ok(M: int, N: int, lda: int, ldb: int) -> bool:
    return _PREC[0] >= 2 and M % 4 == 0 and N % 4 == 0 and 4 <= M <= (1 << 18) and 4 <= N <= (1 << 18) and lda % 4 == 0 and ldb % 4 == 0


def pick(t: torch.Tensor, packed: Optional[torch.Tensor], ok: bool):
    return (packed, True) if (ok and packed is not None) else (t, False)


def weight_T(w2d: torch.Tensor, owner: torch.Tensor) -> torch.Tensor:
    rows, cols = w2d.shape
    src = _contig(w2d)
    im, fresh = _wimage(owner, "T2", WJ_TRANSPOSE, src, (rows, cols, 0),
                        lambda: torch.empty(cols, rows, dtype=torch.float32, device=owner.device))
    if fresh:
        check(lib.glf_transpose2d(_p(src), _p(im.dst), rows, cols, 1, _stream()), "transpose2d")
    return im.dst


def tap_major_T(weight: torch.Tensor) -> torch.Tensor:
    co, ci, kh, kw = weight.shape
    src = _contig(weight.detach())
    taps = kh * kw
    mk = lambda: torch.empty(taps, ci, co, dtype=torch.float32, device=weight.device)
    if taps == 1:
        im, fresh = _wimage(weight, "tapT", WJ_TRANSPOSE, src, (co, ci, 0), mk)
        if fresh:
            check(lib.glf_transpose2d(_p(src), _p(im.dst), co, ci, 1, _stream()), "transpose2d")
        return im.dst
    im, fresh = _wimage(weight, "tapT", WJ_TAP_MAJOR_T, src, (co, ci, taps), mk)
    if fresh:
        check(lib.glf_oihw_to_tap_major_t(_p(src), _p(im.dst), co, ci, taps, _stream()), "oihw_to_tap_major_t")
    return im.dst


def tap_major(weight: torch.Tensor) -> torch.Tensor:
    co, ci, kh, kw = weight.shape
    if kh * kw == 1:
        return _contig(weight.detach()).view(1, co, ci)
    src = _contig(weight.detach())
    im, fresh = _wimage(weight, "tap", WJ_TAP_MAJOR, src, (co, ci, kh * kw),
                        lambda: torch.empty(kh * kw, co, ci, dtype=torch.float32, device=weight.device))
    if fresh:
        check(lib.glf_oihw_to_tap_major(_p(src), _p(im.dst), co, ci, kh * kw, _stream()), "oihw_to_tap_major")
    return im.dst


_rect_cache = {}


def rect_fraction(gather: int, hd: int, wd: int, hs: int, ws: int, kh: int, kw: int, pad: int, dil: int, mask: int) -> float:
    key = (gather, hd, wd, hs, ws, kh, kw, pad, dil, mask)
    f = _rect_cache.get(key)
    if f is None:
        tot, n = 0, 0
        for t in range(kh * kw):
            if not (mask >> t) & 1:
                continue
            ky, kx = divmod(t, kw)
            oy = pad - ky * dil if gather == 1 else ky * dil - pad
            ox = pad - kx * dil if gather == 1 else kx * dil - pad
            rh = max(0, min(hs + oy, hd) - max(oy, 0))
            rw = max(0, min(ws + ox, wd) - max(ox, 0))
            tot += rh * rw
            n += 1
        f = tot / max(1, n * hd * wd)
        _rect_cache[key] = f
    return f


RECT_THRESHOLD = {"fwd": 0.8, "dgrad": 0.8, "wgrad": 0.8, "dgrad_f16x3": 0.35, "region": 0.8}


def region_mode(taps: int, kh: int, stride: int, pad: int, dil: int, h: int, w: int, ho: int, wo: int, k: int, frac: float) -> bool:
    return (_PREC[0] >= 2 and taps == 9 and kh == 3 and stride == 1 and pad == dil and h == ho and w == wo
            and k % 32 == 0 and frac < RECT_THRESHOLD["region"])


def _rect_thr(which: str) -> float:
    if which == "dgrad" and _PREC[0] >= 2:
# ... 1608 lines not shown
```

### include/glfusion.h

```cpp
#ifndef GLFUSION_H
#define GLFUSION_H

#include <stddef.h>
#include <stdint.h>

#ifdef __cplusplus
extern "C" {
#endif

typedef void* glf_stream_t;

typedef enum {
    GLF_OK = 0,
    GLF_ERR_BAD_SHAPE = -1,
    GLF_ERR_UNSUPPORTED = -2,
    GLF_ERR_WORKSPACE = -3,
    GLF_ERR_LAUNCH = -4,
    GLF_ERR_NULL = -5
} glf_status;

typedef enum { GLF_DT_F32 = 0, GLF_DT_BF16 = 1 } glf_dtype;

const char* glf_last_error(void);
int glf_abi_version(void);
int glf_init(void);
int glf_set_precision(int mode);
int glf_get_precision(void);
size_t glf_sizeof_gemm_params(void);

typedef struct {
    int32_t M, N, K;
    int32_t lda, ldb, ldc;
    int32_t taps;
    uint32_t tap_mask;
    int64_t tap_stride_b;
    int32_t gather;
    int32_t n_img, hs, ws, hd, wd, kh, kw, stride, pad, dil;
    int32_t batch;
    int64_t batch_stride_a, batch_stride_b, batch_stride_c;
    float alpha;
    int32_t accumulate;
    int32_t split;
    int32_t rect;
    const float* amax_a;
    const float* amax_b;
    float* amax_c;
    double* colstats;
    float* workspace;
    int64_t workspace_bytes;
    int32_t a_presplit;
    int32_t b_presplit;
    int32_t precision;
    float* colmax;
    int32_t c_dtype;
    int32_t reserved0;
    int32_t c_oihw;
    int32_t foreign_tap;
    const float* foreign_src;
    int64_t foreign_ld;
    int32_t nseg;
    int32_t seg_kx;
    int32_t* seg;
} glf_gemm_params;
#define GLF_TN_OIHW_MAX_TAPS 9
#define GLF_SEG_MAX 28
#define GLF_SEG_MAX_REGIONS 49
#define GLF_SEG_ROW_TILE 256

int glf_gemm_nt_seg_plan(int32_t n_img, int32_t h, int32_t w, int32_t nseg, const int32_t* seg, int32_t* regions,
                         int32_t* n_regions, int64_t* row_tiles);

int glf_amax(const float* x, int64_t rows, int cols, int64_t ld, float* out, glf_stream_t stream);
int glf_split_f16_packed(const float* x, int64_t rows, int cols, int64_t ld, const float* amax, float* out, int64_t ldo,
                         glf_stream_t stream);

int glf_gemm_nt(const float* A, const float* B, const float* bias, float* C,
                const glf_gemm_params* p, glf_stream_t stream);
int glf_gemm_nn(const float* A, const float* B, const float* bias, float* C,
                const glf_gemm_params* p, glf_stream_t stream);
int glf_gemm_tn(const float* A, const float* B, float* C,
                const glf_gemm_params* p, glf_stream_t stream);
size_t glf_gemm_tn_workspace_bytes(const glf_gemm_params* p);

typedef struct {
    const float* shift;
    const float* residual;
    int64_t ld_res;
    int32_t relu;
    int32_t reserved0;
} glf_gemm_epilogue;
int glf_gemm_nt_epilogue(const float* A, const float* B, float* C, const glf_gemm_params* p, const glf_gemm_epilogue* e,
                         glf_stream_t stream);

int glf_s16_gemm_nt(const void* A, const void* B, const float* bias, void* C, const glf_gemm_params* p, glf_stream_t stream);
int glf_s16_gemm_tn(const void* A, const void* B, void* C, const glf_gemm_params* p, glf_stream_t stream);
size_t glf_s16_gemm_tn_workspace_bytes(const glf_gemm_params* p);
typedef struct {
    const float* shift;
    const void* residual;
    int64_t ld_res;
    int32_t relu;
    int32_t reserved;
} glf_s16_gemm_epilogue;
int glf_s16_gemm_nt_epilogue(const void* A, const void* B, void* C, const glf_gemm_params* p, const glf_s16_gemm_epilogue* e,
                             glf_stream_t stream);

typedef struct {
    int32_t n, h, w, cin, cout, kh, kw, stride, pad, dil;
    int32_t precision;
    const float* amax_x;
    const float* amax_w;
    const float* amax_dy;
    float* amax_out;
    double* colstats;
} glf_conv_params;
typedef struct {
    int32_t ho, wo;
    int32_t M, N, K;
    int32_t taps, kept_taps;
    uint32_t tap_mask;
    int32_t plain;
    int32_t rect;
    int32_t split;
    int32_t zero_fill;
    int32_t colstats_ok;
    int64_t workspace_bytes;
} glf_conv_plan;
int glf_conv2d_plan(const glf_conv_params* p, int pass , glf_conv_plan* plan);
int glf_conv2d_fwd(const float* x, const float* w_tap, const float* bias, float* y, const glf_conv_params* p, glf_stream_t s);
int glf_conv2d_fwd_folded(const float* x, const float* w_tap_folded, const float* shift, const float* residual, int64_t ld_res,
                          int relu, float* y, const glf_conv_params* p, glf_stream_t s);
int glf_conv2d_dgrad(const float* dy, const float* w_tap, const float* w_tap_t, float* dx, const glf_conv_params* p, glf_stream_t s);
int glf_conv2d_wgrad(const float* dy, const float* x, float* dw_tap, float* workspace, int64_t workspace_bytes,
                     const glf_conv_params* p, glf_stream_t s);

typedef struct {
    int32_t frames, L, ci;
    int64_t ldq, ldk, ldv;
    int64_t ldy;
    int64_t lddy;
    int64_t ldd;
} glf_attn_params;
int glf_attn_softmax_fwd(const float* theta, const float* phi, const float* g, float* y, float* lse,
                         const glf_attn_params* p, glf_stream_t stream);
int glf_attn_softmax_bwd(const float* theta, const float* phi, const float* g, const float* y, const float* dy, const float* lse,
                         float* dtheta, float* dphi, float* dg, float* dsum_ws, const glf_attn_params* p, glf_stream_t stream);
int glf_s16_attn_softmax_fwd(const void* theta, const void* phi, const void* g, void* y, float* lse,
                             const glf_attn_params* p, glf_stream_t stream);
int glf_s16_attn_softmax_bwd(const void* theta, const void* phi, const void* g, const void* y, const void* dy,
                             const float* lse, void* dtheta, void* dphi, void* dg, float* dsum_ws,
                             const glf_attn_params* p, glf_stream_t stream);

typedef struct {
    int32_t frames, L, ci;
    int32_t reserved0;
    int64_t ldg;
    int64_t ldy;
// ... 115 lines not shown
} glf_tpavi_params;
size_t glf_sizeof_tpavi_params(void);
size_t glf_s16_tpavi_workspace_bytes(const glf_tpavi_params* p, int pass);
int glf_s16_tpavi_fwd(const void* x, const void* w_qkv, const float* b_qkv, const void* w_z, const float* b_z,
                      const float* bn_gamma, const float* bn_beta, float* bn_running_mean, float* bn_running_var,
                      int64_t* num_batches_tracked, const float* ln_gamma, const float* ln_beta, void* z,
                      void* qkv, void* att_t, void* y, void* wz, float* bn_mean, float* bn_invstd, float* row_mean, float* row_rstd,
                      const glf_tpavi_params* p, void* workspace, size_t workspace_bytes, glf_stream_t stream);
int glf_s16_tpavi_bwd(const void* dz, const void* x, const void* qkv, const void* att_t, const void* y, const void* wz,
                      const float* bn_mean, const float* bn_invstd, const float* row_mean, const float* row_rstd,
                      const void* w_qkv_t, const void* w_z_t, const float* bn_gamma, const float* bn_beta, const float* ln_gamma,
                      void* dx, float* dw_qkv, float* db_qkv, float* dw_z, float* db_z, float* dbn_gamma, float* dbn_beta,
                      float* dln_gamma, float* dln_beta, const glf_tpavi_params* p, void* workspace, size_t workspace_bytes,
                      glf_stream_t stream);

int glf_stem7x7_fwd(const float* x, const float* w, const float* bias, float* y,
                    int n, int h, int wdt, int cout, int pad, glf_stream_t s);
int glf_stem7x7_bn_relu_pool(const float* x, const float* w, const float* bias, const float* mean, const float* invstd,
                             const float* gamma, const float* beta, float* y, int n, int h, int wdt, int cout, int pad,
                             float* amax_out, glf_stream_t s);
size_t glf_stem7x7_wgrad_workspace(int n, int h, int wdt, int cout, int pad);
int glf_stem7x7_wgrad(const float* x, const float* dy, float* dw, float* db, float* partial,
                      int n, int h, int wdt, int cout, int pad, glf_stream_t s);

size_t glf_bn_workspace(int rows, int c);
int glf_bn_stats(const float* x, int ldx, int rows, int c, float eps, float momentum,
                 float* mean, float* invstd, float* running_mean, float* running_var,
                 int64_t* num_batches_tracked ,
                 double* workspace, glf_stream_t s);
int glf_bn_stats_from_sums(const double* sums, int rows, int c, float eps, float momentum, float* mean, float* invstd,
                           float* running_mean, float* running_var, int64_t* num_batches_tracked, glf_stream_t s);
int glf_bn_replay_running(const float* mean, const float* invstd, int rows, int c, float eps, float momentum,
                          float* running_mean, float* running_var, int64_t* num_batches_tracked, glf_stream_t s);
int glf_bn_eval_coeffs(const float* running_mean, const float* running_var, float eps,
                       float* mean, float* invstd, int c, glf_stream_t s);
int glf_bn_apply(const float* x, int ldx, const float* residual, int ldr, float* y, int ldy,
                 const float* mean, const float* invstd, const float* gamma, const float* beta,
                 int rows, int c, int relu, float* amax_out, uint8_t* relu_mask, glf_stream_t s);
int glf_bn_apply_from_sums(const float* x, int ldx, const float* residual, int ldr, float* y, int ldy, const double* sums,
                           int rows, int c, float eps, float momentum, const float* gamma, const float* beta,
                           float* mean, float* invstd, float* running_mean, float* running_var, int64_t* num_batches_tracked,
                           int relu, float* amax_out, uint8_t* relu_mask, const float* colmax, glf_stream_t s);
int glf_bn_bwd(const float* dy, int lddy, const float* x, int ldx, const float* y, int ldy,
               const float* mean, const float* invstd, const float* gamma, const float* beta ,
               float* dx, int lddx, float* dres, int lddres, float* dgamma, float* dbeta,
               int rows, int c, int relu, int training, double* workspace, float* amax_out, int packed_dx,
               const uint8_t* relu_mask , const float* dy2, int lddy2,
               double* fused_sums ,
               glf_stream_t s);

int glf_maxpool3x3s2_fwd(const float* x, float* y, uint8_t* idx, int n, int h, int w, int c, glf_stream_t s);
int glf_maxpool3x3s2_bwd(const float* dy, const uint8_t* idx, float* dx, int n, int h, int w, int c, glf_stream_t s);
int glf_avgpool_fwd(const float* x, float* y, int n, int p, int c, glf_stream_t s);
int glf_bcast_rows_fwd(const float* x, float* y, int ldy, int n, int p, int c, glf_stream_t s);
int glf_sum_rows_fwd(const float* dy, int lddy, float* dx, float scale, int n, int p, int c, glf_stream_t s);
int glf_bcast_rows_scaled(const float* x, float* y, int ldy, float scale, int n, int p, int c, glf_stream_t s);
int glf_bcast_rows_add(const float* x, float* y, int ldy, float scale, int n, int p, int c, glf_stream_t s);
int glf_relu_fwd(const float* x, float* y, int64_t numel, glf_stream_t s);
int glf_relu_bwd(const float* dy, const float* y, float* dx, int64_t numel, glf_stream_t s);
int glf_dropout(const float* x, float* y, int64_t numel, float p, uint64_t seed, const uint64_t* step_counter, glf_stream_t s);
int glf_amax_combine(const float* a, const float* b, float scale, int sum, float* out, glf_stream_t s);
int glf_counter_add(uint64_t* counter, uint64_t inc, glf_stream_t s);
int glf_gate_fwd(const float* cls, int ncls, const float* ctr, const float* f, float* y, float* a,
                 int32_t* argmax, float weight, int rows, int c, glf_stream_t s);
int glf_gate_bwd(const float* dy, const float* f, const float* cls, int ncls, const float* ctr,
                 const float* a, const int32_t* argmax, float weight,
                 float* df, float* dcls, float* dctr, int rows, int c, glf_stream_t s);
int glf_copy_frames(const float* src, int64_t src_fs, float* dst, int64_t dst_fs,
                    int n, int64_t inner, glf_stream_t s);
int glf_copy_frames_split(const float* src, int64_t src_fs, float* dst, float* dst_packed, int64_t dst_fs, int n, int64_t inner,
                          const float* amax, glf_stream_t s);
int glf_add_frames(const float* a, int64_t a_fs, const float* b, int64_t b_fs, float* dst, int64_t dst_fs,
                   int n, int64_t inner, glf_stream_t s);
int glf_add_n(const float* const* inputs, int k, float* out, int64_t numel, glf_stream_t s);
int glf_bn_res_ln_fwd(const float* w, const float* x, const float* bn_mean, const float* bn_invstd,
                      const float* bn_gamma, const float* bn_beta, const float* ln_gamma,
                      const float* ln_beta, float ln_eps, float* z, float* row_mean, float* row_rstd,
                      int rows, int c, float* amax_out, glf_stream_t s);
int glf_bn_res_ln_bwd(const float* dz, const float* w, const float* x, const float* bn_mean,
                      const float* bn_invstd, const float* bn_gamma, const float* bn_beta,
                      const float* ln_gamma, const float* row_mean, const float* row_rstd,
                      float* du, float* dln_gamma, float* dln_beta, int rows, int c,
                      double* workspace, glf_stream_t s);
int glf_softmax_rows(float* x, int64_t rows, int cols, glf_stream_t s);
int glf_softmax_rows_bwd(const float* p, float* dp_inout, int64_t rows, int cols, glf_stream_t s);
int glf_softmax_rows_ld(float* x, int64_t rows, int cols, int ld, glf_stream_t s);
int glf_softmax_rows_bwd_ld(const float* p, float* dp_inout, int64_t rows, int cols, int ld, glf_stream_t s);
int glf_bilinear_up_fwd(const float* x, float* y, int n, int h, int w, int c, int ho, int wo, glf_stream_t s);
int glf_bilinear_up_bwd(const float* dy, float* dx, int n, int h, int w, int c, int ho, int wo, glf_stream_t s);
int glf_bce_logits_sum(const float* x, const float* t, double* loss_out, float* dx, float grad_scale,
                       const float* grad_scale_dev, int64_t numel, glf_stream_t s);
int glf_overlap_counts(const float* logits, const float* target, int64_t* counts, int64_t numel, glf_stream_t s);
int glf_colsum(const float* dy, int lddy, float* db, int rows, int c, double* workspace, glf_stream_t s);

int glf_adam_step(const int64_t* table, int n_rows, double lr, double beta1, double beta2, double eps,
                  double weight_decay, int64_t step, glf_stream_t s);
int glf_sgd_step(const int64_t* table, int n_rows, double lr, double momentum, double dampening, double weight_decay,
                 int nesterov, int first, glf_stream_t s);
int glf_grad_sumsq(const int64_t* table, int n_rows, double* partials, glf_stream_t s);
int glf_grad_clip_coef(const double* partials, int n, double max_norm, float* record, int64_t* skipped, glf_stream_t s);
int glf_adam_step_clipped(const int64_t* table, int n_rows, double lr, double beta1, double beta2, double eps,
                          double weight_decay, int64_t step, const float* record, glf_stream_t s);
int glf_sgd_step_clipped(const int64_t* table, int n_rows, double lr, double momentum, double dampening, double weight_decay,
                         int nesterov, int first, const float* record, glf_stream_t s);
int glf_grad_scale(const int64_t* table, int n_rows, const float* record, glf_stream_t s);

int glf_seg_cycle(const float* feat, int T, int F, int target_region, int cyc_off, int chunk_size, float temperature,
                  int start0, int n_starts, int stride, float weight, int soft_label, float* loss_out, float* dfeat,
                  glf_stream_t s);
int glf_axpby(const float* x, const float* y, float* out, float a, float b, int64_t numel, glf_stream_t s);
int glf_scale(const float* x, float* y, int64_t numel, float scale, const float* scale_dev, glf_stream_t s);
int glf_prepare_frames(const float* img, const float* lab, float* out_img, float* out_mask, int H0, int W0, int T,
                       int resize, int out_h, int out_w, int off_y, int off_x, const int* class_to_channel, float img_div,
                       glf_stream_t s);
int glf_overlap_counts_nchw(const float* logits, const float* target, int64_t* counts, int n, int c, int64_t hw, glf_stream_t s);
int glf_zero(void* p, int64_t bytes, glf_stream_t s);

#ifdef __cplusplus
}
#endif
#endif
```

### profiles/ubench/kstats_groups.py

```python
#!/usr/bin/env python3
import csv
import re
import sys

rows = list(csv.DictReader(open(sys.argv[1])))
steps = float(sys.argv[2]) if len(sys.argv) > 2 else 1.0
groups = [("NT contractions", r"gemm_rows|s16_rows_kernel|gemm_skinny"), ("TN contractions (wgrad)", r"gemm_tn|s16_tn_kernel"), ("tn_reduce", r"tn_reduce"),
          ("BN bwd reduce", r"colreduce_kernel<.*OpBnBwd|bnbwd_reduce"), ("BN bwd apply", r"bn_bwd_apply|bnbwd_apply"), ("BN apply", r"bn_apply_kernel|bn_apply_sums"),
          ("BN stats / finalize", r"colreduce_kernel<.*OpStats|bn_stats_finalize|sum_finalize|bnbwd_finalize"),
          ("other column reduces", r"colreduce"), ("add_n (fan-in)", r"add_n"), ("split_packed", r"split_packed"),
          ("weights refresh", r"weights_refresh"), ("bn_res_ln", r"bn_res_ln"), ("stem", r"stem"), ("maxpool", r"maxpool"),
          ("at::native", r"at::native|elementwise_kernel|vectorized"), ("amax", r"amax_kernel")]
tot = {g: [0.0, 0] for g, _ in groups}
rest, rest_n, allt = {}, 0, 0.0
for r in rows:
    name, t, n = r["Name"], float(r["TotalDurationNs"]) / 1e6, int(r["Calls"])
    if re.search(r"spin_kernel|probe_mfma", name):
        aids = aids + t if "aids" in dir() else t
        continue
    allt += t
    for g, pat in groups:
        if re.search(pat, name):
            tot[g][0] += t; tot[g][1] += n
            break
    else:
        k = re.sub(r"\(anonymous namespace\)::|void ", "", name)[:50]
        rest[k] = rest.get(k, 0.0) + t
print(f"total kernel time {allt / steps:.1f} ms/step over {steps:g} steps (bench.py's spin / probe kernels left out: {(aids if 'aids' in dir() else 0.0) / steps:.1f} ms/step)")
for g, _ in groups:
    if tot[g][1]:
        print(f"  {g:28s} {tot[g][0] / steps:8.2f} ms/step  {tot[g][1] / steps:8.1f} launches/step")
for k, t in sorted(rest.items(), key=lambda kv: -kv[1])[:12]:
    print(f"  {k:50s} {t / steps:8.2f} ms/step")
```

Before: 17.51 clips/s.

## Fuse tail backward reductions and fold bias colsum into split-packed pass

Adds a fused bn_res_ln backward kernel that walks dz/w/x once. In that single pass it produces du plus the LN and BN column sums, and one merged finalize kernel reduces them. It also adds a split_packed_colsum kernel that computes the bias-gradient column sum while splitting the activation into fp16 hi/lo, so the separate colsum read of dqkv is gone. The intent is to cut memory passes and kernel launches in the transformer-tail backward. The cost is more complex kernels with higher register and shared-memory use, which may reduce occupancy, and a changed reduction order.

```diff
diff --git a/gl-fusion_amd/csrc/gemm_common.h b/gl-fusion_amd/csrc/gemm_common.h
--- a/gl-fusion_amd/csrc/gemm_common.h
+++ b/gl-fusion_amd/csrc/gemm_common.h
@@ -55,6 +55,8 @@
 int launch_rows_f16s4(const GemmArgs& a, dim3 grid, bool gather, int nprod, hipStream_t s);
 int launch_amax(const float* x, long long rows, int cols, long long ld, int vec, float* out, hipStream_t s);
 int launch_split_packed(const float* x, long long rows, int cols, long long ld, const float* amax, float* out, long long ldo, hipStream_t s);
+int launch_split_packed_colsum(const float* x, int rows, int cols, long long ld, const float* amax, float* out, long long ldo,
+                               float* colsum, double* workspace, hipStream_t s);
 float* amax_scratch(int n, hipStream_t s);
 const float* zero_page();
 bool f16s_rows_ok(const GemmArgs& a);
diff --git a/gl-fusion_amd/csrc/gemm_f16s.hip b/gl-fusion_amd/csrc/gemm_f16s.hip
--- a/gl-fusion_amd/csrc/gemm_f16s.hip
+++ b/gl-fusion_amd/csrc/gemm_f16s.hip
@@ -1285,6 +1285,79 @@
     }
 }
 
+
+constexpr int SC_FLUSH = 64;
+__global__ __launch_bounds__(256) void split_packed_colsum_kernel(const float* __restrict__ x, int rows, int cols4, long long ld,
+                                                                  const float* __restrict__ amax, float* __restrict__ out, long long ldo,
+                                                                  int tpr, int cblocks, int slices, double* __restrict__ partial) {
+    __shared__ double sh[256 * 4];
+    float sc, inv;
+    pow2_scale(amax, sc, inv);
+    const int rpp = 256 / tpr;
+    const int ct = threadIdx.x % tpr, rl = threadIdx.x / tpr;
+    const int cb = blockIdx.x % cblocks, slice = blockIdx.x / cblocks;
+    const int per = (rows + slices - 1) / slices;
+    const int r0 = slice * per, r1 = min(rows, r0 + per);
+    const int cc = cb * tpr + ct, c0 = cc * 4;
+    const bool live = cc < cols4 && rl < rpp;
+    double d0 = 0, d1 = 0, d2 = 0, d3 = 0;
+    if (live) {
+        float4 acc = make_float4(0.f, 0.f, 0.f, 0.f);
+        int n = 0;
+        auto emit = [&](long long row, const float4 v) __attribute__((always_inline)) {
+            const SplitH sp = split4h(v, sc);
+            const float2 h = __builtin_bit_cast(float2, sp.h), l = __builtin_bit_cast(float2, sp.l);
+            *reinterpret_cast<float4*>(out + row * ldo + c0) = make_float4(h.x, h.y, l.x, l.y);
+            acc.x += v.x; acc.y += v.y; acc.z += v.z; acc.w += v.w;
+        };
+        auto fold = [&]() __attribute__((always_inline)) {
+            d0 += (double)acc.x; d1 += (double)acc.y; d2 += (double)acc.z; d3 += (double)acc.w;
+            acc = make_float4(0.f, 0.f, 0.f, 0.f); n = 0;
+        };
+        int r = r0 + rl;
+        for (; r + 3 * rpp < r1; r += 4 * rpp) {
+            float4 qv[4];
+#pragma unroll
+            for (int u = 0; u < 4; ++u) qv[u] = *reinterpret_cast<const float4*>(x + (long long)(r + u * rpp) * ld + c0);
+            __builtin_amdgcn_sched_barrier(0);
+#pragma unroll
+            for (int u = 0; u < 4; ++u) emit(r + u * rpp, qv[u]);
+            n += 4;
+            if (n >= SC_FLUSH) fold();
+        }
+        for (; r < r1; r += rpp) emit(r, *reinterpret_cast<const float4*>(x + (long long)r * ld + c0));
+        fold();
+    }
+    sh[threadIdx.x * 4 + 0] = d0; sh[threadIdx.x * 4 + 1] = d1; sh[threadIdx.x * 4 + 2] = d2; sh[threadIdx.x * 4 + 3] = d3;
+    __syncthreads();
+    if (rl == 0 && cc < cols4) {
+        for (int k = 1; k < rpp; ++k) {
+            const int o = (k * tpr + ct) * 4;
+            d0 += sh[o]; d1 += sh[o + 1]; d2 += sh[o + 2]; d3 += sh[o + 3];
+        }
+        double* pd = partial + (long long)slice * (cols4 * 4) + c0;
+        pd[0] = d0; pd[1] = d1; pd[2] = d2; pd[3] = d3;
+    }
+}
+
+__global__ __launch_bounds__(256) void split_colsum_finalize(const double* __restrict__ partial, int slices, int cols, float* __restrict__ colsum) {
+    __shared__ double sh[256];
+    const int cx = threadIdx.x % 16, lane = threadIdx.x / 16;
+    const int ch = blockIdx.x * 16 + cx;
+    double s = 0, s1 = 0;
+    if (ch < cols) {
+        int i = lane;
+        for (; i + 16 < slices; i += 32) { s += partial[(long long)i * cols + ch]; s1 += partial[(long long)(i + 16) * cols + ch]; }
+        if (i < slices) s += partial[(long long)i * cols + ch];
+        s += s1;
+    }
+    sh[threadIdx.x] = s;
+    __syncthreads();
+    if (lane != 0 || ch >= cols) return;
+    for (int l = 1; l < 16; ++l) s += sh[threadIdx.x + l * 16];
+    colsum[ch] = (float)s;
+}
+
 }
 
 namespace glf {
@@ -1295,6 +1368,25 @@
     if (blocks > 8192) blocks = 8192;
     hipLaunchKernelGGL(split_packed_kernel, dim3((unsigned)blocks), dim3(256), 0, s, x, rows, cols / 4, ld, amax, out, ldo);
     return check_launch("split_f16_packed");
+}
+
+int launch_split_packed_colsum(const float* x, int rows, int cols, long long ld, const float* amax, float* out, long long ldo,
+                               float* colsum, double* workspace, hipStream_t s) {
+    const int c4 = cols / 4;
+    const int tpr = c4 >= 64 ? 64 : (c4 < 16 ? c4 : 16);
+    const int rpp = 256 / tpr;
+    const int cblocks = (c4 + tpr - 1) / tpr;
+    long long sl = (long long)num_cus() * 8 / cblocks;
+    const int smax = (rows + rpp - 1) / rpp;
+    if (sl > smax) sl = smax;
+    if (sl > 1024) sl = 1024;
+    if (sl < 1) sl = 1;
+    const int slices = (int)sl;
+    hipLaunchKernelGGL(split_packed_colsum_kernel, dim3((unsigned)slices * (unsigned)cblocks), dim3(256), 0, s, x, rows, c4, ld, amax, out, ldo,
+                       tpr, cblocks, slices, workspace);
+    if (int rc = check_launch("split_f16_packed_colsum")) return rc;
+    hipLaunchKernelGGL(split_colsum_finalize, dim3((cols + 15) / 16), dim3(256), 0, s, workspace, slices, cols, colsum);
+    return check_launch("split_colsum_finalize");
 }
 
 int init_gemm_f16s_attrs() {
diff --git a/gl-fusion_amd/csrc/gemm_f32.hip b/gl-fusion_amd/csrc/gemm_f32.hip
--- a/gl-fusion_amd/csrc/gemm_f32.hip
+++ b/gl-fusion_amd/csrc/gemm_f32.hip
@@ -822,6 +822,17 @@
     return glf::launch_split_packed(x, rows, cols, ld, amax, out, ldo, glf::S(stream));
 }
 
+extern "C" int glf_split_f16_packed_colsum(const float* x, int rows, int cols, int64_t ld, const float* amax, float* out, int64_t ldo,
+                                           float* colsum, double* workspace, glf_stream_t stream) {
+    if (int rc = glf::ensure_init()) return rc;
+    GLF_REQUIRE(x && amax && out && colsum && workspace, GLF_ERR_NULL, "split_f16_packed_colsum: null argument");
+    GLF_REQUIRE(rows > 0 && cols > 0 && cols % 4 == 0 && ld % 4 == 0 && ldo % 4 == 0 && ld >= cols && ldo >= cols, GLF_ERR_BAD_SHAPE,
+                "split_f16_packed_colsum: cols and the row strides must be multiples of 4");
+    GLF_REQUIRE(aligned16(x) && aligned16(out), GLF_ERR_BAD_SHAPE, "split_f16_packed_colsum: x and out must be 16-byte aligned");
+    GLF_REQUIRE(out != x, GLF_ERR_BAD_SHAPE, "split_f16_packed_colsum: out must not alias x");
+    return glf::launch_split_packed_colsum(x, rows, cols, ld, amax, out, ldo, colsum, workspace, glf::S(stream));
+}
+
 constexpr int SK_COLS = 2;
 __global__ __launch_bounds__(256) void gemm_skinny_nt_kernel(const float* __restrict__ A, const float* __restrict__ B, const float* __restrict__ bias,
                                                             float* __restrict__ C, int M, int N, int K, int lda, int ldb, int ldc, float alpha,
diff --git a/gl-fusion_amd/csrc/norm.hip b/gl-fusion_amd/csrc/norm.hip
--- a/gl-fusion_amd/csrc/norm.hip
+++ b/gl-fusion_amd/csrc/norm.hip
@@ -340,7 +340,7 @@
     }
 }
 
-__global__ __launch_bounds__(256) void sum_finalize(const double* __restrict__ partial, int slices, int c, float* out_a, float* out_b) {
+__device__ __forceinline__ void sum_finalize_body(const double* __restrict__ partial, int slices, int c, float* out_a, float* out_b) {
     __shared__ double sh[512];
     const int cx = threadIdx.x % FIN_CH, lane = threadIdx.x / FIN_CH;
     const int ch = blockIdx.x * FIN_CH + cx;
@@ -350,11 +350,14 @@
     if (out_a) out_a[ch] = (float)s;
     if (out_b) out_b[ch] = (float)q;
 }
-
-__global__ __launch_bounds__(256) void bnbwd_finalize(const double* __restrict__ partial, const float* __restrict__ pmax, int slices, int c,
-                                                      const float* __restrict__ gamma, const float* __restrict__ invstd, float inv_n,
-                                                      int training, float* out_a, float* out_b, float* __restrict__ bound,
-                                                      float* __restrict__ keep) {
+__global__ __launch_bounds__(256) void sum_finalize(const double* __restrict__ partial, int slices, int c, float* out_a, float* out_b) {
+    sum_finalize_body(partial, slices, c, out_a, out_b);
+}
+
+__device__ __forceinline__ void bnbwd_finalize_body(const double* __restrict__ partial, const float* __restrict__ pmax, int slices, int c,
+                                                    const float* __restrict__ gamma, const float* __restrict__ invstd, float inv_n,
+                                                    int training, float* out_a, float* out_b, float* __restrict__ bound,
+                                                    float* __restrict__ keep) {
     __shared__ double sh[512];
     __shared__ float shm[512];
     const int cx = threadIdx.x % FIN_CH, lane = threadIdx.x / FIN_CH;
@@ -386,7 +389,20 @@
     if (keep) { keep[ch] = (float)s; keep[c + ch] = (float)q; }
     const float k = fabsf(gamma[ch] * invstd[ch]);
     const float b = 1.0001f * k * (training ? mg + inv_n * (fabsf((float)s) + mx * fabsf((float)q)) : mg);
-    if (b > 0.f && b < 3.0e38f) atomicMax(reinterpret_cast<unsigned*>(bound), __float_as_uint(b));
+    if (bound && b > 0.f && b < 3.0e38f) atomicMax(reinterpret_cast<unsigned*>(bound), __float_as_uint(b));
+}
+__global__ __launch_bounds__(256) void bnbwd_finalize(const double* __restrict__ partial, const float* __restrict__ pmax, int slices, int c,
+                                                      const float* __restrict__ gamma, const float* __restrict__ invstd, float inv_n,
+                                                      int training, float* out_a, float* out_b, float* __restrict__ bound,
+                                                      float* __restrict__ keep) {
+    bnbwd_finalize_body(partial, pmax, slices, c, gamma, invstd, inv_n, training, out_a, out_b, bound, keep);
+}
+__global__ __launch_bounds__(256) void tail_bwd_finalize(const double* __restrict__ partial, const float* __restrict__ pmax, int slices, int c,
+                                                         const float* __restrict__ gamma, const float* __restrict__ invstd, float inv_n,
+                                                         int training, float* dln_g, float* dln_b, float* dbn_b, float* dbn_g,
+                                                         float* __restrict__ bound, float* __restrict__ keep) {
+    if (blockIdx.y == 0) sum_finalize_body(partial, slices, c, dln_g, dln_b);
+    else bnbwd_finalize_body(partial + (size_t)2 * slices * c, pmax, slices, c, gamma, invstd, inv_n, training, dbn_b, dbn_g, bound, keep);
 }
 
 __global__ void bn_replay_kernel(const float* __restrict__ mean, const float* __restrict__ invstd, int rows, float eps, float momentum,
@@ -779,6 +795,168 @@
     }
 }
 
+__device__ __forceinline__ float rounded(float p) { asm volatile("" : "+v"(p)); return p; }
+constexpr int TA_R = 3;
+constexpr int TA_FLUSH = 15;
+constexpr int TA_MAX_SLICES = 512;
+
+inline int tail_slices(int rows) {
+    int s = (rows + 4 * TA_R - 1) / (4 * TA_R);
+    int cap = 2 * num_cus();
+    if (cap > TA_MAX_SLICES) cap = TA_MAX_SLICES;
+    return s < 1 ? 1 : (s > cap ? cap : s);
+}
+
+__global__ __launch_bounds__(256, 2) void bn_res_ln_bwd_sums_kernel(const float* __restrict__ dz, const float* __restrict__ w,
+                                                                    const float* __restrict__ x, Coef bn, const float* __restrict__ ln_g,
+                                                                    const float* __restrict__ row_mean, const float* __restrict__ row_rstd,
+                                                                    float* __restrict__ du, int rows, int c, int slices,
+                                                                    double* __restrict__ partial, float* __restrict__ pmax) {
+    __shared__ float sT[TA_R][2][7][64];
+    __shared__ double sD[32][256];
+    const int tid = threadIdx.x, lane = tid & 63, q = tid >> 6;
+    const int c4 = c >> 2;
+    const int slice = blockIdx.x;
+    const int per = (rows + slices - 1) / slices;
+    const int r0 = slice * per, r1 = min(rows, r0 + per);
+    const float4 zero4 = make_float4(0.f, 0.f, 0.f, 0.f);
+    int ch[2]; bool lv[2];
+    float4 mu[2], is[2], ga[2], be[2], lg[2];
+    float4 sa[2], sb[2], mg[2], mx[2];
+#pragma unroll
+    for (int j = 0; j < 2; ++j) {
+        const int cc = lane + 64 * (2 * q + j);
+        lv[j] = cc < c4; ch[j] = cc * 4;
+        mu[j] = is[j] = ga[j] = be[j] = lg[j] = zero4;
+        if (lv[j]) {
+            mu[j] = *reinterpret_cast<const float4*>(bn.mean + ch[j]);
+            is[j] = *reinterpret_cast<const float4*>(bn.invstd + ch[j]);
+            ga[j] = *reinterpret_cast<const float4*>(bn.gamma + ch[j]);
+            be[j] = *reinterpret_cast<const float4*>(bn.beta + ch[j]);
+            lg[j] = *reinterpret_cast<const float4*>(ln_g + ch[j]);
+        }
+        sa[j] = sb[j] = mg[j] = mx[j] = zero4;
+    }
+#pragma unroll
+    for (int k = 0; k < 32; ++k) sD[k][tid] = 0.0;
+    auto flush = [&]() __attribute__((always_inline)) {
+#pragma unroll
+        for (int j = 0; j < 2; ++j) {
+            const float4 v[2] = {sa[j], sb[j]};
+#pragma unroll
+            for (int st = 0; st < 2; ++st) {
+                sD[16 + st * 8 + j * 4 + 0][tid] += (double)v[st].x; sD[16 + st * 8 + j * 4 + 1][tid] += (double)v[st].y;
+                sD[16 + st * 8 + j * 4 + 2][tid] += (double)v[st].z; sD[16 + st * 8 + j * 4 + 3][tid] += (double)v[st].w;
+            }
+            sa[j] = sb[j] = zero4;
+        }
+    };
+    int pending = 0;
+    for (int rb = r0; rb < r1; rb += TA_R) {
+        float4 gz[TA_R][2], uh[TA_R][2], wh[TA_R][2];
+        float rm[TA_R], rs[TA_R];
+#pragma unroll
+        for (int u = 0; u < TA_R; ++u) {
+            const int row = rb + u;
+            const bool ok = row < r1;
+            const long long base = (long long)row * c;
+#pragma unroll
+            for (int j = 0; j < 2; ++j) {
+                gz[u][j] = uh[u][j] = wh[u][j] = zero4;
+                if (ok && lv[j]) {
+                    gz[u][j] = *reinterpret_cast<const float4*>(dz + base + ch[j]);
+                    wh[u][j] = *reinterpret_cast<const float4*>(w + base + ch[j]);
+                    uh[u][j] = *reinterpret_cast<const float4*>(x + base + ch[j]);
+                }
+            }
+            rm[u] = ok ? row_mean[row] : 0.f;
+            rs[u] = ok ? row_rstd[row] : 0.f;
+        }
+        __builtin_amdgcn_sched_barrier(0);
+#pragma unroll
+        for (int u = 0; u < TA_R; ++u) {
+            const bool ok = rb + u < r1;
+            const float mean = rm[u], rstd = rs[u];
+            float t1[2], t2[2];
+#pragma unroll
+            for (int j = 0; j < 2; ++j) {
+                const float4 d = gz[u][j], ww = wh[u][j], xx = uh[u][j];
+                const float4 wn = make_float4((ww.x - mu[j].x) * is[j].x, (ww.y - mu[j].y) * is[j].y, (ww.z - mu[j].z) * is[j].z, (ww.w - mu[j].w) * is[j].w);
+                float4 uu = make_float4(__builtin_fmaf(wn.x, ga[j].x, be[j].x) + xx.x, __builtin_fmaf(wn.y, ga[j].y, be[j].y) + xx.y,
+                                        __builtin_fmaf(wn.z, ga[j].z, be[j].z) + xx.z, __builtin_fmaf(wn.w, ga[j].w, be[j].w) + xx.w);
+                uu = make_float4((uu.x - mean) * rstd, (uu.y - mean) * rstd, (uu.z - mean) * rstd, (uu.w - mean) * rstd);
+                const float4 g = make_float4(rounded(d.x * lg[j].x), rounded(d.y * lg[j].y), rounded(d.z * lg[j].z), rounded(d.w * lg[j].w));
+                const float4 pr = make_float4(rounded(g.x * uu.x), rounded(g.y * uu.y), rounded(g.z * uu.z), rounded(g.w * uu.w));
+                t1[j] = (g.x + g.y) + (g.z + g.w);
+                t2[j] = (j == 1 && q == 0) ? __builtin_fmaf(g.x, uu.x, pr.y) + __builtin_fmaf(g.z, uu.z, pr.w) : (pr.x + pr.y) + (pr.z + pr.w);
+                sD[j * 4 + 0][tid] += (double)(d.x * uu.x); sD[j * 4 + 1][tid] += (double)(d.y * uu.y);
+                sD[j * 4 + 2][tid] += (double)(d.z * uu.z); sD[j * 4 + 3][tid] += (double)(d.w * uu.w);
+                sD[8 + j * 4 + 0][tid] += (double)d.x; sD[8 + j * 4 + 1][tid] += (double)d.y;
+                sD[8 + j * 4 + 2][tid] += (double)d.z; sD[8 + j * 4 + 3][tid] += (double)d.w;
+                if (ok && lv[j]) {
+                    mx[j].x = fmaxf(mx[j].x, fabsf(wn.x)); mx[j].y = fmaxf(mx[j].y, fabsf(wn.y));
+                    mx[j].z = fmaxf(mx[j].z, fabsf(wn.z)); mx[j].w = fmaxf(mx[j].w, fabsf(wn.w));
+                }
+                gz[u][j] = g; uh[u][j] = uu; wh[u][j] = wn;
+            }
+            if (q == 0) {
+                float p1 = 0.f, p2 = 0.f;
+                if (lv[0]) { p1 += t1[0]; p2 += t2[0]; }
+                if (lv[1]) { p1 += t1[1]; p2 += t2[1]; }
+                sT[u][0][0][lane] = p1; sT[u][1][0][lane] = p2;
+            } else {
+                sT[u][0][2 * q - 1][lane] = lv[0] ? t1[0] : 0.f; sT[u][1][2 * q - 1][lane] = lv[0] ? t2[0] : 0.f;
+                sT[u][0][2 * q][lane] = lv[1] ? t1[1] : 0.f;     sT[u][1][2 * q][lane] = lv[1] ? t2[1] : 0.f;
+            }
+        }
+        __syncthreads();
+        float m1[TA_R], m2[TA_R];
+#pragma unroll
+        for (int u = 0; u < TA_R; ++u) {
+            float s1 = sT[u][0][0][lane], s2 = sT[u][1][0][lane];
+#pragma unroll
+            for (int k = 1; k < 7; ++k) { s1 += sT[u][0][k][lane]; s2 += sT[u][1][k][lane]; }
+            m1[u] = wave_sum(s1) / c; m2[u] = wave_sum(s2) / c;
+        }
+        __syncthreads();
+#pragma unroll
+        for (int u = 0; u < TA_R; ++u) {
+            const int row = rb + u;
+            if (row < r1) {
+                const float rstd = rs[u];
+                const long long base = (long long)row * c;
+#pragma unroll
+                for (int j = 0; j < 2; ++j)
+                    if (lv[j]) {
+                        const float4 g = gz[u][j], uu = uh[u][j], wn = wh[u][j];
+                        const float4 o = make_float4(rstd * __builtin_fmaf(-m2[u], uu.x, g.x - m1[u]), rstd * __builtin_fmaf(-m2[u], uu.y, g.y - m1[u]),
+                                                     rstd * __builtin_fmaf(-m2[u], uu.z, g.z - m1[u]), rstd * __builtin_fmaf(-m2[u], uu.w, g.w - m1[u]));
+                        *reinterpret_cast<float4*>(du + base + ch[j]) = o;
+                        sa[j].x += o.x; sa[j].y += o.y; sa[j].z += o.z; sa[j].w += o.w;
+                        sb[j].x += o.x * wn.x; sb[j].y += o.y * wn.y; sb[j].z += o.z * wn.z; sb[j].w += o.w * wn.w;
+                        mg[j].x = fmaxf(mg[j].x, fabsf(o.x)); mg[j].y = fmaxf(mg[j].y, fabsf(o.y));
+                        mg[j].z = fmaxf(mg[j].z, fabsf(o.z)); mg[j].w = fmaxf(mg[j].w, fabsf(o.w));
+                    }
+            }
+        }
+        pending += TA_R;
+        if (pending + TA_R > TA_FLUSH) { flush(); pending = 0; }
+    }
+    flush();
+#pragma unroll
+    for (int j = 0; j < 2; ++j)
+        if (lv[j]) {
+#pragma unroll
+            for (int st = 0; st < 4; ++st) {
+                double* pd = partial + ((long long)st * slices + slice) * c + ch[j];
+                pd[0] = sD[st * 8 + j * 4 + 0][tid]; pd[1] = sD[st * 8 + j * 4 + 1][tid];
+                pd[2] = sD[st * 8 + j * 4 + 2][tid]; pd[3] = sD[st * 8 + j * 4 + 3][tid];
+            }
+            *reinterpret_cast<float4*>(pmax + (long long)slice * c + ch[j]) = mg[j];
+            *reinterpret_cast<float4*>(pmax + (long long)(slices + slice) * c + ch[j]) = mx[j];
+        }
+}
+
 template <class Op>
 int launch_colreduce(Op op, int rows, int c, double* ws, hipStream_t s) {
     const int slices = n_slices_c(rows, c);
@@ -883,7 +1061,7 @@
     if (int rc = glf::ensure_init()) return rc;
     GLF_REQUIRE(dy && x && mean && invstd && gamma && dx && (workspace || fused_sums), GLF_ERR_NULL, "bn_bwd: null argument");
     if (relu_mask) y = nullptr;
-    GLF_REQUIRE(!packed_dx || amax_out, GLF_ERR_NULL, "bn_bwd: packed_dx needs amax_out (a zeroed device float that receives the bound the image is scaled with)");
+    GLF_REQUIRE(!packed_dx || packed_dx == 4 || amax_out, GLF_ERR_NULL, "bn_bwd: packed_dx needs amax_out (a zeroed device float that receives the bound the image is scaled with)");
     GLF_REQUIRE(!relu || y || beta || relu_mask, GLF_ERR_NULL, "bn_bwd: relu != 0 needs relu_mask, y (the forward output) or beta (to recompute its sign from x)");
     GLF_REQUIRE(rows > 0, GLF_ERR_BAD_SHAPE, "bn_bwd: rows must be > 0");
     REQ_C4(c); REQ_AL(dy, "dy"); REQ_AL(x, "x"); REQ_AL(dx, "dx"); REQ_LD(lddy, "lddy"); REQ_LD(ldx, "ldx"); REQ_LD(lddx, "lddx");
@@ -894,10 +1072,10 @@
     const ColGrid ag = col_grid(rows, c);
     BwdApply ap{dy, lddy, x, ldx, y, ldy, Coef{mean, invstd, gamma, beta}, nullptr, nullptr, dx, lddx, dres, lddres,
                 rows, c, ag.tpr, ag.cblocks, ag.slices, training, 1.0f / (float)rows,
-                amax_out, packed_dx, relu_mask, dy2, lddy2, nullptr, nullptr, nullptr, nullptr};
+                amax_out, packed_dx == 4 ? 0 : packed_dx, relu_mask, dy2, lddy2, nullptr, nullptr, nullptr, nullptr};
     const int phase = packed_dx >= 2 ? packed_dx : 0;
-    GLF_REQUIRE(packed_dx >= 0 && packed_dx <= 3, GLF_ERR_BAD_SHAPE, "bn_bwd: packed_dx must be 0 .. 3");
-    GLF_REQUIRE(!phase || (workspace && fused_sums), GLF_ERR_NULL, "bn_bwd: packed_dx = 2 / 3 needs the workspace and fused_sums (2 c floats kept from half 2 to half 3)");
+    GLF_REQUIRE(packed_dx >= 0 && packed_dx <= 4, GLF_ERR_BAD_SHAPE, "bn_bwd: packed_dx must be 0 .. 4");
+    GLF_REQUIRE(!phase || (workspace && fused_sums), GLF_ERR_NULL, "bn_bwd: packed_dx = 2 / 3 / 4 needs the workspace and fused_sums (2 c floats kept from half 2 to half 3)");
     GLF_REQUIRE(phase != 2 || (dgamma && dbeta), GLF_ERR_NULL, "bn_bwd: packed_dx = 2 needs dgamma and dbeta");
     float* keep = phase ? reinterpret_cast<float*>(fused_sums) : (float*)nullptr;
     if (!phase && fused_sums && c <= APPLY_MAX_C) {
@@ -928,7 +1106,7 @@
     float* sums = reinterpret_cast<float*>(workspace + (size_t)2 * slices * c);
     float* s_dy = dbeta ? dbeta : sums;
     float* s_dyx = dgamma ? dgamma : sums + c;
-    if (phase == 3) {
+    if (phase >= 3) {
         s_dy = keep; s_dyx = keep + c;
     } else if (packed_dx) {
         float* pmax = reinterpret_cast<float*>(workspace + (size_t)2 * slices * c + (size_t)2 * c);
@@ -993,3 +1171,26 @@
     hipLaunchKernelGGL(sum_finalize, dim3((c + FIN_CH - 1) / FIN_CH), dim3(256), 0, glf::S(s), workspace, n_slices_c(rows, c), c, dln_gamma, dln_beta);
     return glf::check_launch("ln_param_finalize");
 }
+
+extern "C" int glf_bn_res_ln_bwd_sums(const float* dz, const float* w, const float* x, const float* bn_mean,
+                                      const float* bn_invstd, const float* bn_gamma, const float* bn_beta,
+                                      const float* ln_gamma, const float* row_mean, const float* row_rstd,
+                                      float* du, float* dln_gamma, float* dln_beta, float* dbn_gamma, float* dbn_beta,
+                                      float* bn_sums, float* amax_out, int rows, int c, int training,
+                                      double* workspace, glf_stream_t s) {
+    if (int rc = glf::ensure_init()) return rc;
+    GLF_REQUIRE(dz && w && x && bn_mean && bn_invstd && bn_gamma && bn_beta && ln_gamma && row_mean && row_rstd && du &&
+                dln_gamma && dln_beta && dbn_gamma && dbn_beta && bn_sums && workspace, GLF_ERR_NULL, "bn_res_ln_bwd_sums: null argument");
+    GLF_REQUIRE(rows > 0, GLF_ERR_BAD_SHAPE, "bn_res_ln_bwd_sums: rows must be > 0");
+    REQ_C4(c); GLF_REQUIRE(c <= 64 * 4 * LN_NV, GLF_ERR_UNSUPPORTED, "bn_res_ln: C must be <= %d", 64 * 4 * LN_NV);
+    REQ_AL(dz, "dz"); REQ_AL(w, "w"); REQ_AL(x, "x"); REQ_AL(du, "du");
+    GLF_REQUIRE(du != dz && du != w && du != x, GLF_ERR_BAD_SHAPE, "bn_res_ln_bwd_sums: du must not alias dz, w or x");
+    const int slices = tail_slices(rows);
+    float* pmax = reinterpret_cast<float*>(workspace + (size_t)4 * slices * c);
+    hipLaunchKernelGGL(bn_res_ln_bwd_sums_kernel, dim3(slices), dim3(256), 0, glf::S(s), dz, w, x, Coef{bn_mean, bn_invstd, bn_gamma, bn_beta},
+                       ln_gamma, row_mean, row_rstd, du, rows, c, slices, workspace, pmax);
+    if (int rc = glf::check_launch("bn_res_ln_bwd_sums")) return rc;
+    hipLaunchKernelGGL(tail_bwd_finalize, dim3((c + FIN_CH - 1) / FIN_CH, 2), dim3(256), 0, glf::S(s), workspace, pmax, slices, c, bn_gamma,
+                       bn_invstd, 1.0f / (float)rows, training, dln_gamma, dln_beta, dbn_beta, dbn_gamma, amax_out, bn_sums);
+    return glf::check_launch("tail_bwd_finalize");
+}
diff --git a/gl-fusion_amd/fusion.py b/gl-fusion_amd/fusion.py
--- a/gl-fusion_amd/fusion.py
+++ b/gl-fusion_amd/fusion.py
@@ -11,11 +11,13 @@
 
 from ._lib import AttnPairParams, AttnParams, check, lib
 from .ops import (_chk, _contig, _p, _stream, _tn_split, _ws, _wimage, _registry, WJ_COPY, stats_slot, bnbwd_slot, amax_of, amax_slot, colsum, gemm, set_amax, split_mode,
-                  transpose2d, weight_T, weight_packed, nt_presplit_ok, tn_presplit_ok, act_packed, packed_hit, pick, zeros, _ones4)
+                  transpose2d, weight_T, weight_packed, nt_presplit_ok, tn_presplit_ok, act_packed, act_packed_colsum, packed_hit, pick, zeros,
+                  _ones4)
 
 
 FUSED_SOFTMAX = os.environ.get("GLF_FUSED_SOFTMAX", "1") != "0"
 EXACT_KCHUNK = int(os.environ.get("GLF_EXACT_KCHUNK", "256"))
+TAIL_BWD_FUSED = os.environ.get("GLF_TAIL_BWD_FUSED", "1") != "0"
 _gemm = gemm
 
 
@@ -387,11 +389,15 @@
     dWcat = torch.empty(c3, c, **G.f32)
     am_dq = amax_of(dqkv)
     ok = tn_presplit_ok(c3, c, c3, c)
+    dbcat = None
+    if ok and TAIL_BWD_FUSED and rows < (1 << 31) // c3:
+        _, dbcat = act_packed_colsum(dqkv, am_dq, rows, c3)
     dq_a, pa = pick(dqkv, act_packed(dqkv, am_dq, True) if ok else None, ok)
     am_x = x_packed[1] if x_packed is not None else amax_of(x)
     xb, pb = pick(x, x_packed[0] if x_packed is not None else None, ok)
     gemm("tn", dq_a, xb, dWcat, M=c3, N=c, K=rows, lda=c3, ldb=c, ldc=c, split=sp, amax_a=am_dq, amax_b=am_x, a_packed=pa, b_packed=pb)
-    dbcat = colsum(dqkv, rows, c3)
+    if dbcat is None:
+        dbcat = colsum(dqkv, rows, c3)
     if _split_dgrad(G):
         WcatT = weight_T(Wcat, Wcat)
         am_wc = amax_of(Wcat)
@@ -443,18 +449,28 @@
     du = torch.empty(rows, c, **G.f32)
     dln_g = torch.empty(c, **G.f32)
     dln_b = torch.empty(c, **G.f32)
-    check(lib.glf_bn_res_ln_bwd(_p(dz), _p(wz), _p(x), _p(mean), _p(invstd), _p(bn_g), _p(bn_b), _p(ln_g), _p(rmu), _p(rrs),
-                                _p(du), _p(dln_g), _p(dln_b), rows, c, _p(_ws(rows, c, dev)), _stream()), "bn_res_ln_bwd")
     split = _split_dgrad(G)
     dwz = torch.empty(rows, c, **G.f32)
     am_dwz_slot = amax_slot(dev)
     dbn_g = torch.empty(c, **G.f32)
     dbn_b = torch.empty(c, **G.f32)
     dwz_pk = bool(training and split and am_dwz_slot is not None and nt_presplit_ok(c, c, c) and tn_presplit_ok(c, ci, c, ci))
-    fused = bnbwd_slot(c, dev) if c <= 4096 else None
-    check(lib.glf_bn_bwd(_p(du), c, _p(wz), c, None, c, _p(mean), _p(invstd), _p(bn_g), None, _p(dwz), c, None, c,
-                         _p(dbn_g), _p(dbn_b), rows, c, 0, int(training), None if fused is not None else _p(_ws(rows, c, dev)), _p(am_dwz_slot),
-                         int(dwz_pk), None, None, 0, _p(fused), _stream()), "bn_bwd")
+    if TAIL_BWD_FUSED:
+        keep = torch.empty(2 * c, **G.f32)
+        ws = _ws(rows, c, dev)
+        check(lib.glf_bn_res_ln_bwd_sums(_p(dz), _p(wz), _p(x), _p(mean), _p(invstd), _p(bn_g), _p(bn_b), _p(ln_g), _p(rmu), _p(rrs),
+                                         _p(du), _p(dln_g), _p(dln_b), _p(dbn_g), _p(dbn_b), _p(keep), _p(am_dwz_slot) if dwz_pk else None,
+                                         rows, c, int(training), _p(ws), _stream()), "bn_res_ln_bwd_sums")
+        check(lib.glf_bn_bwd(_p(du), c, _p(wz), c, None, c, _p(mean), _p(invstd), _p(bn_g), None, _p(dwz), c, None, c,
+                             None, None, rows, c, 0, int(training), _p(ws), _p(am_dwz_slot), 3 if dwz_pk else 4, None, None, 0, _p(keep),
+                             _stream()), "bn_bwd")
+    else:
+        check(lib.glf_bn_res_ln_bwd(_p(dz), _p(wz), _p(x), _p(mean), _p(invstd), _p(bn_g), _p(bn_b), _p(ln_g), _p(rmu), _p(rrs),
+                                    _p(du), _p(dln_g), _p(dln_b), rows, c, _p(_ws(rows, c, dev)), _stream()), "bn_res_ln_bwd")
+        fused = bnbwd_slot(c, dev) if c <= 4096 else None
+        check(lib.glf_bn_bwd(_p(du), c, _p(wz), c, None, c, _p(mean), _p(invstd), _p(bn_g), None, _p(dwz), c, None, c,
+                             _p(dbn_g), _p(dbn_b), rows, c, 0, int(training), None if fused is not None else _p(_ws(rows, c, dev)), _p(am_dwz_slot),
+                             int(dwz_pk), None, None, 0, _p(fused), _stream()), "bn_bwd")
     set_amax(dwz, am_dwz_slot)
     sp = _tn_split(rows, c, ci, 1)
     if not split_mode():
diff --git a/gl-fusion_amd/ops.py b/gl-fusion_amd/ops.py
--- a/gl-fusion_amd/ops.py
+++ b/gl-fusion_amd/ops.py
@@ -674,6 +674,20 @@
     return pk
 
 
+def act_packed_colsum(t: torch.Tensor, amax: Optional[torch.Tensor], rows: int, cols: int):
+    if not presplit_ok(t, amax) or packed_hit(t, amax) is not None:
+        return None, None
+    pk = torch.empty_like(t)
+    db = torch.empty(cols, dtype=torch.float32, device=t.device)
+    check(lib.glf_split_f16_packed_colsum(_p(t), rows, cols, cols, _p(amax), _p(pk), cols, _p(db), _p(_ws(rows, cols, t.device)), _stream()),
+          "split_f16_packed_colsum")
+    try:
+        t._glf_packed = (t._version, t.data_ptr(), amax, pk, torch.cuda.current_stream() if STREAMS else None)
+    except AttributeError:
+        pass
+    return pk, db
+
+
 def nt_presplit_ok(K: int, lda: int, ldb: int) -> bool:
     return _PREC[0] >= 2 and K % 32 == 0 and 32 <= K <= (1 << 18) and lda % 4 == 0 and ldb % 4 == 0
 
diff --git a/include/glfusion.h b/include/glfusion.h
--- a/include/glfusion.h
+++ b/include/glfusion.h
@@ -73,6 +73,8 @@
 int glf_amax(const float* x, int64_t rows, int cols, int64_t ld, float* out, glf_stream_t stream);
 int glf_split_f16_packed(const float* x, int64_t rows, int cols, int64_t ld, const float* amax, float* out, int64_t ldo,
                          glf_stream_t stream);
+int glf_split_f16_packed_colsum(const float* x, int rows, int cols, int64_t ld, const float* amax, float* out, int64_t ldo,
+                                float* colsum, double* workspace, glf_stream_t stream);
 
 int glf_gemm_nt(const float* A, const float* B, const float* bias, float* C,
                 const glf_gemm_params* p, glf_stream_t stream);
@@ -354,6 +356,12 @@
                       const float* ln_gamma, const float* row_mean, const float* row_rstd,
                       float* du, float* dln_gamma, float* dln_beta, int rows, int c,
                       double* workspace, glf_stream_t s);
+int glf_bn_res_ln_bwd_sums(const float* dz, const float* w, const float* x, const float* bn_mean,
+                           const float* bn_invstd, const float* bn_gamma, const float* bn_beta,
+                           const float* ln_gamma, const float* row_mean, const float* row_rstd,
+                           float* du, float* dln_gamma, float* dln_beta, float* dbn_gamma, float* dbn_beta,
+                           float* bn_sums, float* amax_out , int rows, int c, int training,
+                           double* workspace, glf_stream_t s);
 int glf_softmax_rows(float* x, int64_t rows, int cols, glf_stream_t s);
 int glf_softmax_rows_bwd(const float* p, float* dp_inout, int64_t rows, int cols, glf_stream_t s);
 int glf_softmax_rows_ld(float* x, int64_t rows, int cols, int ld, glf_stream_t s);
diff --git a/profiles/ubench/kstats_groups.py b/profiles/ubench/kstats_groups.py
--- a/profiles/ubench/kstats_groups.py
+++ b/profiles/ubench/kstats_groups.py
@@ -7,7 +7,7 @@
 steps = float(sys.argv[2]) if len(sys.argv) > 2 else 1.0
 groups = [("NT contractions", r"gemm_rows|s16_rows_kernel|gemm_skinny"), ("TN contractions (wgrad)", r"gemm_tn|s16_tn_kernel"), ("tn_reduce", r"tn_reduce"),
           ("BN bwd reduce", r"colreduce_kernel<.*OpBnBwd|bnbwd_reduce"), ("BN bwd apply", r"bn_bwd_apply|bnbwd_apply"), ("BN apply", r"bn_apply_kernel|bn_apply_sums"),
-          ("BN stats / finalize", r"colreduce_kernel<.*OpStats|bn_stats_finalize|sum_finalize|bnbwd_finalize"),
+          ("BN stats / finalize", r"colreduce_kernel<.*OpStats|bn_stats_finalize|sum_finalize|bnbwd_finalize|tail_bwd_finalize|split_colsum_finalize"),
           ("other column reduces", r"colreduce"), ("add_n (fan-in)", r"add_n"), ("split_packed", r"split_packed"),
           ("weights refresh", r"weights_refresh"), ("bn_res_ln", r"bn_res_ln"), ("stem", r"stem"), ("maxpool", r"maxpool"),
           ("at::native", r"at::native|elementwise_kernel|vectorized"), ("amax", r"amax_kernel")]
diff --git a/profiles/ubench/tail_bwd_probe.py b/profiles/ubench/tail_bwd_probe.py
--- /dev/null
+++ b/profiles/ubench/tail_bwd_probe.py
@@ -0,0 +1,67 @@
+import sys, os, json
+sys.path.insert(0, os.getcwd())
+import torch
+from glfusion_amd._lib import lib
+DEV = torch.device("cuda:0")
+
+def timeit(fn, n=10, warm=3):
+    for _ in range(warm): fn()
+    ts = []
+    for _ in range(n):
+        a, b = torch.cuda.Event(enable_timing=True), torch.cuda.Event(enable_timing=True)
+        a.record(); fn(); b.record(); torch.cuda.synchronize()
+        ts.append(a.elapsed_time(b))
+    ts.sort()
+    return 0.5 * (ts[len(ts) // 2] + ts[(len(ts) - 1) // 2])
+
+out = {}
+new = hasattr(lib.load(), "glf_bn_res_ln_bwd_sums")
+for rows in (150528, 37632):
+    c, c3 = 2048, 3072
+    T = rows * c * 4 / 1e9
+    g = torch.Generator(device=DEV).manual_seed(1)
+    dz = torch.randn(rows, c, device=DEV, generator=g); w = torch.randn(rows, c, device=DEV, generator=g); x = torch.randn(rows, c, device=DEV, generator=g)
+    v = {k: torch.rand(c, device=DEV, generator=g) + 0.5 for k in ("mean", "invstd", "gamma", "beta", "ln_g", "ln_b")}
+    z = torch.empty(rows, c, device=DEV); rmu = torch.empty(rows, device=DEV); rrs = torch.empty(rows, device=DEV)
+    P = lambda t: t.data_ptr()
+    assert lib.glf_bn_res_ln_fwd(P(w), P(x), P(v["mean"]), P(v["invstd"]), P(v["gamma"]), P(v["beta"]), P(v["ln_g"]), P(v["ln_b"]), 1e-5, P(z), P(rmu), P(rrs), rows, c, None, None) == 0
+    del z
+    du = torch.empty(rows, c, device=DEV); dwz = torch.empty(rows, c, device=DEV)
+    o = [torch.empty(c, device=DEV) for _ in range(4)]; keep = torch.empty(2 * c, device=DEV)
+    ws = torch.empty(int(lib.glf_bn_workspace(rows, c3)), dtype=torch.float64, device=DEV)
+    am = torch.zeros(1, device=DEV)
+    slot = torch.zeros(3 * c + 2, dtype=torch.float64, device=DEV)
+    res = {}
+    def ab():
+        assert lib.glf_bn_res_ln_bwd(P(dz), P(w), P(x), P(v["mean"]), P(v["invstd"]), P(v["gamma"]), P(v["beta"]), P(v["ln_g"]), P(rmu), P(rrs), P(du), P(o[0]), P(o[1]), rows, c, P(ws), None) == 0
+    res["a+b glf_bn_res_ln_bwd (du + LN colreduce + finalize)"] = (timeit(ab), 7 * T)
+    def cd():
+        slot.zero_(); am.zero_()
+        assert lib.glf_bn_bwd(P(du), c, P(w), c, None, c, P(v["mean"]), P(v["invstd"]), P(v["gamma"]), None, P(dwz), c, None, c, P(o[2]), P(o[3]), rows, c, 0, 1, None, P(am), 1, None, None, 0, P(slot), None) == 0
+    res["c+d glf_bn_bwd fused form packed (atomic reduce + apply)"] = (timeit(cd), 5 * T)
+    def c2():
+        am.zero_()
+        assert lib.glf_bn_bwd(P(du), c, P(w), c, None, c, P(v["mean"]), P(v["invstd"]), P(v["gamma"]), None, P(dwz), c, None, c, P(o[2]), P(o[3]), rows, c, 0, 1, P(ws), P(am), 2, None, None, 0, P(keep), None) == 0
+    res["(c') glf_bn_bwd packed_dx=2 (two-stage reduce + finalize)"] = (timeit(c2), 2 * T)
+    def d3():
+        assert lib.glf_bn_bwd(P(du), c, P(w), c, None, c, P(v["mean"]), P(v["invstd"]), P(v["gamma"]), None, P(dwz), c, None, c, None, None, rows, c, 0, 1, P(ws), P(am), 3, None, None, 0, P(keep), None) == 0
+    res["d glf_bn_bwd packed_dx=3 (apply alone)"] = (timeit(d3), 3 * T)
+    if new:
+        def A():
+            am.zero_()
+            assert lib.glf_bn_res_ln_bwd_sums(P(dz), P(w), P(x), P(v["mean"]), P(v["invstd"]), P(v["gamma"]), P(v["beta"]), P(v["ln_g"]), P(rmu), P(rrs), P(du), P(o[0]), P(o[1]), P(o[2]), P(o[3]), P(keep), P(am), rows, c, 1, P(ws), None) == 0
+        res["A glf_bn_res_ln_bwd_sums (walk + finalize)"] = (timeit(A), 4 * T)
+    del dz, w, x, du, dwz
+    dq = torch.randn(rows, c3, device=DEV, generator=g); pk = torch.empty_like(dq); s = torch.empty(c3, device=DEV)
+    amq = dq.abs().max().reshape(1)
+    Q = rows * c3 * 4 / 1e9
+    res["e glf_split_f16_packed dqkv"] = (timeit(lambda: lib.glf_split_f16_packed(P(dq), rows, c3, c3, P(amq), P(pk), c3, None)), 2 * Q)
+    res["f glf_colsum dqkv"] = (timeit(lambda: lib.glf_colsum(P(dq), c3, P(s), rows, c3, P(ws), None)), Q)
+    if new:
+        res["E glf_split_f16_packed_colsum dqkv"] = (timeit(lambda: lib.glf_split_f16_packed_colsum(P(dq), rows, c3, c3, P(amq), P(pk), c3, P(s), P(ws), None)), 2 * Q)
+    del dq, pk
+    for k, (ms, gb) in res.items():
+        print(f"rows {rows:6d}  {k:62s} {ms:7.3f} ms  {gb / ms * 1e3 / 1e3:6.2f} TB/s ({gb:.2f} GB)", flush=True)
+    out[rows] = {k: [ms, gb] for k, (ms, gb) in res.items()}
+    torch.cuda.empty_cache()
+json.dump(out, open(sys.argv[1], "w"), indent=1)
```

Result: faster. 17.72 clips/s, median of 6 (+1.2%).
